# CMB-BNU/PloidyFrost

Hardware: AMD Instinct MI355X
Metric: unitigs/s through superbubble+SeqAlign (k=25, z=8) (higher is better)
Workload: dtype u64

## Files before the change

ploidyfrost_amd/csrc/pf_call.hip:

```cpp
#include "pf_call_kernels.hpp"
#include "pf_scan.hpp"

using namespace pf;

#define PF_HIP(call)                                                                         \
    do {                                                                                     \
        hipError_t e_ = (call);                                                              \
        if (e_ != hipSuccess) {                                                              \
            pf::CtxErr{ctx} = std::string(#call) + ": " + hipGetErrorString(e_);                   \
            return PF_ERR_HIP;                                                               \
        }                                                                                    \
    } while (0)

#define PF_TRY(call) do { const int s_ = (call); if (s_ != PF_OK) return s_; } while (0)

using namespace pf_call;

struct Need { DevBuf *buf; size_t bytes; };
static int need(pf_ctx *ctx, const char *who, std::initializer_list<Need> list) {
    for (const Need &n : list)
        if (!n.buf->ensure(n.bytes)) { pf::CtxErr{ctx} = std::string(who) + ": out of device memory"; return PF_ERR_HIP; }
    return PF_OK;
}

namespace pf {

void call_state_create(pf_ctx *ctx) { (void)state_of(ctx); }
void call_destroy(pf_ctx *ctx) {
    if (!ctx->call) return;
    ctx->call->release_all();
    delete ctx->call;
    ctx->call = nullptr;
}
void call_invalidate(pf_ctx *ctx) {
    if (!ctx->call) return;
    ctx->call->have_cov = false;
    ctx->call->have_state = false;
    ctx->call->n_sides = ctx->call->n_tasks = 0;
}

}

namespace pf {
int call_state_arrays(pf_ctx *ctx, uint8_t **flags, uint32_t **plus, uint32_t **minus) {
    if (!ctx->d_seq || !ctx->has_adj) { pf::CtxErr{ctx} = "T1 state: graph and adjacency first"; return PF_ERR_ARG; }
    CallState *S = state_of(ctx);
    const size_t N = ctx->N;
    if (!S->flags.ensure(N + 1) || !S->plus.ensure(N * 4) || !S->minus.ensure(N * 4)) { pf::CtxErr{ctx} = "T1 state: out of device memory"; return PF_ERR_HIP; }
    *flags = S->flags.as<uint8_t>();
    *plus = S->plus.as<uint32_t>();
    *minus = S->minus.as<uint32_t>();
    S->have_state = false;
    return PF_OK;
}
void call_state_resident(pf_ctx *ctx) {
    CallState *S = state_of(ctx);
    S->have_state = true;
    S->n_sides = S->n_tasks = 0;
}
}

extern "C" {

int pf_format_doubles(pf_ctx *ctx, const double *values, uint64_t n, char *text, uint8_t *len) {
    if (!ctx || (n && (!values || !text || !len))) return PF_ERR_ARG;
    if (n == 0) return PF_OK;
    PF_HIP(hipSetDevice(ctx->device));
    DevTmp<double> dx;
    DevTmp<char> dt;
    DevTmp<uint8_t> dl;
    PF_HIP(dx.alloc(n * 8));
    PF_HIP(dt.alloc(n * 32));
    PF_HIP(dl.alloc(n));
    PF_HIP(hipMemcpyAsync(dx.p, values, n * 8, hipMemcpyDefault, ctx->stream));
    k_format_doubles<<<(unsigned)((n + 255) / 256), 256, 0, ctx->stream>>>(dx.p, n, dt.p, dl.p);
    PF_HIP(hipGetLastError());
    PF_HIP(hipMemcpyAsync(text, dt.p, n * 32, hipMemcpyDefault, ctx->stream));
    PF_HIP(hipMemcpyAsync(len, dl.p, n, hipMemcpyDefault, ctx->stream));
    PF_HIP(hipStreamSynchronize(ctx->stream));
    return PF_OK;
}

int pf_call_set_state(pf_ctx *ctx, const uint8_t *flags, const uint32_t *plus, const uint32_t *minus) {
    if (!ctx || !flags || !plus || !minus) return PF_ERR_ARG;
    if (!ctx->d_seq || !ctx->has_adj) { pf::CtxErr{ctx} = "pf_call_set_state: graph and adjacency first"; return PF_ERR_ARG; }
    PF_HIP(hipSetDevice(ctx->device));
    CallState *S = state_of(ctx);
    const size_t N = ctx->N;
    if (!S->flags.ensure(N + 1) || !S->plus.ensure(N * 4) || !S->minus.ensure(N * 4)) { pf::CtxErr{ctx} = "pf_call_set_state: out of device memory"; return PF_ERR_HIP; }
    PF_HIP(hipMemcpyAsync(S->flags.p, flags, N, hipMemcpyDefault, ctx->stream));
    PF_HIP(hipMemcpyAsync(S->plus.p, plus, N * 4, hipMemcpyDefault, ctx->stream));
    PF_HIP(hipMemcpyAsync(S->minus.p, minus, N * 4, hipMemcpyDefault, ctx->stream));
    PF_HIP(hipStreamSynchronize(ctx->stream));
    S->have_state = true;
    S->n_sides = S->n_tasks = 0;
    return PF_OK;
}

int pf_call_get_state(pf_ctx *ctx, uint8_t *flags, uint32_t *plus, uint32_t *minus) {
    if (!ctx || !ctx->call) return PF_ERR_ARG;
    CallState *S = ctx->call;
    if (!S->have_state) { pf::CtxErr{ctx} = "pf_call_get_state: no T1 state on the device"; return PF_ERR_ARG; }
    PF_HIP(hipSetDevice(ctx->device));
    const size_t N = ctx->N;
    PF_HIP(hipStreamSynchronize(ctx->stream));
    if (flags) PF_HIP(hipMemcpy(flags, S->flags.p, N, hipMemcpyDeviceToHost));
    if (plus) PF_HIP(hipMemcpy(plus, S->plus.p, N * 4, hipMemcpyDeviceToHost));
    if (minus) PF_HIP(hipMemcpy(minus, S->minus.p, N * 4, hipMemcpyDeviceToHost));
    return PF_OK;
}

int pf_call_set_format(pf_ctx *ctx, int reference_mt) {
    if (!ctx) return PF_ERR_ARG;
    state_of(ctx)->mt_format = reference_mt != 0;
    return PF_OK;
}

int pf_superbubble_rows(pf_ctx *ctx, int colored_rule, uint64_t *n_rows, uint64_t *text_len) {
    if (!ctx || !n_rows || !text_len) return PF_ERR_ARG;
    CallState *S = ctx->call;
    if (!S || !S->have_state) { pf::CtxErr{ctx} = "pf_superbubble_rows: pf_call_set_state first"; return PF_ERR_ARG; }
    PF_HIP(hipSetDevice(ctx->device));
    hipStream_t st = ctx->stream;
    const uint32_t N = ctx->N;
    const size_t n1 = (size_t)N + 1;
    if (!S->sb_cnt.ensure(n1 * 4) || !S->sb_base.ensure(n1 * 4) || !S->sb_sizes.ensure(n1 * 4) || !S->sb_offs.ensure(n1 * 8)) {
        pf::CtxErr{ctx} = "pf_superbubble_rows: out of device memory";
        return PF_ERR_HIP;
    }
    SbArgs a;
    a.flags = S->flags.as<uint8_t>(); a.plus = S->plus.as<uint32_t>(); a.minus = S->minus.as<uint32_t>(); a.N = N; a.colored = colored_rule;
    a.first_id = S->mt_format ? 0u : 1u;
    a.row_base = S->sb_base.as<uint32_t>(); a.sizes = S->sb_sizes.as<uint32_t>(); a.offs = S->sb_offs.as<uint64_t>(); a.out = nullptr;
    const unsigned grid = (unsigned)((n1 + 255) / 256);
    k_sb_count<<<grid, 256, 0, st>>>(a, S->sb_cnt.as<uint32_t>());
    if (!S->scan_tmp.ensure(scan_scratch_bytes(n1))) { pf::CtxErr{ctx} = "pf_superbubble_rows: out of device memory"; return PF_ERR_HIP; }
    PF_HIP(scan_exclusive_u32(S->sb_cnt.as<uint32_t>(), S->sb_base.as<uint32_t>(), n1, S->scan_tmp.p, st));
    ctx_begin(ctx, PF_K_CALL_FORMAT);
    k_sb_format<false><<<grid, 256, 0, st>>>(a);
    ctx_end(ctx);
    PF_HIP(scan_exclusive_u32_u64(S->sb_sizes.as<uint32_t>(), S->sb_offs.as<uint64_t>(), n1, S->scan_tmp.p, st));
    uint32_t rows = 0;
    uint64_t len = 0;
    PF_HIP(hipMemcpyAsync(&rows, S->sb_base.as<uint32_t>() + N, 4, hipMemcpyDeviceToHost, st));
    PF_HIP(hipMemcpyAsync(&len, S->sb_offs.as<uint64_t>() + N, 8, hipMemcpyDeviceToHost, st));
    PF_HIP(hipStreamSynchronize(st));
    if (!S->sb_out.ensure(std::max<uint64_t>(len, 16))) { pf::CtxErr{ctx} = "pf_superbubble_rows: out of device memory"; return PF_ERR_HIP; }
    a.out = S->sb_out.as<char>();
    hipStream_t wst = S->copy_stream ? S->copy_stream : st;
    ctx_begin_on(ctx, PF_K_CALL_FORMAT, wst);
    k_sb_format<true><<<grid, 256, 0, wst>>>(a);
    ctx_end_on(ctx, wst);
    PF_HIP(hipGetLastError());
    if (wst == st) PF_HIP(hipStreamSynchronize(st));
    S->sb_len = len;
    *n_rows = rows;
    *text_len = len;
    return PF_OK;
}

int pf_superbubble_fetch(pf_ctx *ctx, char *dst, uint64_t len) {
    if (!ctx || !ctx->call || (len && !dst)) return PF_ERR_ARG;
    CallState *S = ctx->call;
    if (len > S->sb_len) return PF_ERR_ARG;
    if (len == 0) return PF_OK;
    if (hipSetDevice(ctx->device) != hipSuccess || !S->copy_stream) return PF_ERR_HIP;
    size_t tl_at = (size_t)-1;
    (void)ctx_begin_at(ctx, PF_K_COPY_TEXT, S->copy_stream, &tl_at);
    if (hipMemcpyAsync(dst, S->sb_out.p, (size_t)len, hipMemcpyDeviceToHost, S->copy_stream) != hipSuccess) return PF_ERR_HIP;
    ctx_end_at(ctx, tl_at, S->copy_stream);
    if (hipStreamSynchronize(S->copy_stream) != hipSuccess) return PF_ERR_HIP;
    return PF_OK;
}

int pf_call_set_colours(pf_ctx *ctx, uint32_t n_colors, const uint64_t *full_mask, const uint64_t *size_total, const uint32_t *part_first,
                        const uint32_t *part_colour, const uint64_t *part_word, const uint64_t *part_bits, uint64_t n_part, uint64_t n_words) {
    if (!ctx || !ctx->d_seq) { if (ctx) pf::CtxErr{ctx} = "pf_call_set_colours: graph first"; return PF_ERR_ARG; }
    PF_HIP(hipSetDevice(ctx->device));
    CallState *S = state_of(ctx);
    S->n_colors = 0;
    S->have_cov = false;
    if (!n_colors) return PF_OK;
    if (n_colors > PF_MAX_COLORS || n_colors != ctx->n_colors || !full_mask || !size_total || !part_first || (n_part && (!part_colour || !part_word)) ||
        (n_words && !part_bits)) {
        pf::CtxErr{ctx} = "pf_call_set_colours: the colour sets of every unitig, for the colours of the uploaded databases, are required";
        return PF_ERR_ARG;
    }
    const size_t N = ctx->N, CW = (n_colors + 63) / 64;
    if (!S->col_low.ensure((size_t)n_colors * 4) || !S->col_up.ensure((size_t)n_colors * 4) || !S->col_full.ensure(N * CW * 8) || !S->col_size.ensure(N * 8) ||
        !S->part_first.ensure((N + 1) * 4) || !S->part_colour.ensure((n_part + 1) * 4) || !S->part_word.ensure((n_part + 1) * 8) ||
        !S->part_bits.ensure((n_words + 1) * 8)) {
        pf::CtxErr{ctx} = "pf_call_set_colours: out of device memory";
        return PF_ERR_HIP;
    }
    hipStream_t st = ctx->stream;
    PF_HIP(hipMemsetAsync(S->col_low.p, 0, (size_t)n_colors * 4, st));
    PF_HIP(hipMemsetAsync(S->col_up.p, 0xFF, (size_t)n_colors * 4, st));
    PF_HIP(hipMemcpyAsync(S->col_full.p, full_mask, N * CW * 8, hipMemcpyDefault, st));
    PF_HIP(hipMemcpyAsync(S->col_size.p, size_total, N * 8, hipMemcpyDefault, st));
    PF_HIP(hipMemcpyAsync(S->part_first.p, part_first, (N + 1) * 4, hipMemcpyDefault, st));
    if (n_part) {
        PF_HIP(hipMemcpyAsync(S->part_colour.p, part_colour, n_part * 4, hipMemcpyDefault, st));
        PF_HIP(hipMemcpyAsync(S->part_word.p, part_word, n_part * 8, hipMemcpyDefault, st));
    }
    if (n_words) PF_HIP(hipMemcpyAsync(S->part_bits.p, part_bits, n_words * 8, hipMemcpyDefault, st));
    PF_HIP(hipStreamSynchronize(st));
    S->n_colors = n_colors;
    S->col_words = (uint32_t)CW;
    return PF_OK;
}

int pf_call_set_cutoffs(pf_ctx *ctx, uint32_t n_colors, const uint32_t *lower, const uint32_t *upper) {
    if (!ctx || !ctx->call || !ctx->call->n_colors || n_colors != ctx->call->n_colors || !lower || !upper) {
        if (ctx) pf::CtxErr{ctx} = "pf_call_set_cutoffs: pf_call_set_colours first; one (lower, upper) per colour";
        return PF_ERR_ARG;
    }
    PF_HIP(hipSetDevice(ctx->device));
    CallState *S = ctx->call;
    PF_HIP(hipMemcpyAsync(S->col_low.p, lower, (size_t)n_colors * 4, hipMemcpyDefault, ctx->stream));
    PF_HIP(hipMemcpyAsync(S->col_up.p, upper, (size_t)n_colors * 4, hipMemcpyDefault, ctx->stream));
    PF_HIP(hipStreamSynchronize(ctx->stream));
    return PF_OK;
}

int pf_call_coverage(pf_ctx *ctx) {
    if (ctx && ctx->call && ctx->call->n_colors) {
        if (!ctx->d_seq || !ctx->d_ctab) { pf::CtxErr{ctx} = "pf_call_coverage: graph and count tables first"; return PF_ERR_ARG; }
        PF_HIP(hipSetDevice(ctx->device));
        CallState *S = ctx->call;
        const size_t n = (size_t)ctx->N * S->n_colors;
        if (!S->ccov_sum.ensure(n * 8) || !S->ccov_min.ensure(n * 4) || !S->ccov_max.ensure(n * 4) || !S->ccov_miss.ensure(n)) {
            pf::CtxErr{ctx} = "pf_call_coverage: out of device memory";
            return PF_ERR_HIP;
        }
        const int st = pf_unitig_cov_colored(ctx, 0, ctx->N, S->ccov_sum.as<uint64_t>(), S->ccov_min.as<uint32_t>(), S->ccov_max.as<uint32_t>(), S->ccov_miss.as<uint8_t>());
        if (st != PF_OK) return st;
        S->per_strand = false;
        S->have_cov = true;
        return PF_OK;
    }
    if (!ctx || !ctx->d_seq || !ctx->d_tab) { if (ctx) pf::CtxErr{ctx} = "pf_call_coverage: graph and count table first"; return PF_ERR_ARG; }
    PF_HIP(hipSetDevice(ctx->device));
    CallState *S = state_of(ctx);
    const size_t N = ctx->N;
    const int slots = ctx->tab_exact ? 2 : 1;
    if (!S->cov_sum.ensure(N * slots * 8) || !S->cov_min.ensure(N * slots * 4) || !S->cov_miss.ensure(N * slots)) {
        pf::CtxErr{ctx} = "pf_call_coverage: out of device memory";
        return PF_ERR_HIP;
    }
    int st;
    if (!ctx->tab_exact) {
        st = pf_unitig_cov(ctx, 0, (uint32_t)N, S->cov_sum.as<uint64_t>(), S->cov_min.as<uint32_t>(), S->cov_miss.as<uint8_t>());
    } else {
        st = pf_unitig_cov_exact(ctx, 0, (uint32_t)N, 0, S->cov_sum.as<uint64_t>(), S->cov_min.as<uint32_t>(), S->cov_miss.as<uint8_t>());
        if (st == PF_OK || st == PF_ERR_MISSING_KMER)
            st = pf_unitig_cov_exact(ctx, 0, (uint32_t)N, 1, S->cov_sum.as<uint64_t>() + N, S->cov_min.as<uint32_t>() + N, S->cov_miss.as<uint8_t>() + N);
    }
    if (st != PF_OK && st != PF_ERR_MISSING_KMER) return st;
    S->per_strand = ctx->tab_exact;
    S->have_cov = true;
    return PF_OK;
}

int pf_call_scan(pf_ctx *ctx, uint32_t lower, uint32_t upper, uint64_t *n_sides) {
    if (!ctx || !n_sides) return PF_ERR_ARG;
    CallState *S = ctx->call;
    if (!S || !S->have_state || !S->have_cov) { pf::CtxErr{ctx} = "pf_call_scan: pf_call_set_state and pf_call_coverage first"; return PF_ERR_ARG; }
    PF_HIP(hipSetDevice(ctx->device));
    hipStream_t st = ctx->stream;
    const uint32_t N = ctx->N;
    if (!S->side_cnt.ensure(((size_t)N + 1) * 4) || !S->side_base.ensure(((size_t)N + 1) * 4)) { pf::CtxErr{ctx} = "pf_call_scan: out of device memory"; return PF_ERR_HIP; }
    k_call_count_sides<<<(N + 1 + 255) / 256, 256, 0, st>>>(S->flags.as<uint8_t>(), N, S->side_cnt.as<uint32_t>());
    if (!S->scan_tmp.ensure(scan_scratch_bytes((uint64_t)N + 1))) { pf::CtxErr{ctx} = "pf_call_scan: out of device memory"; return PF_ERR_HIP; }
    PF_HIP(scan_exclusive_u32(S->side_cnt.as<uint32_t>(), S->side_base.as<uint32_t>(), (uint64_t)N + 1, S->scan_tmp.p, st));
    uint32_t total = 0;
    PF_HIP(hipMemcpyAsync(&total, S->side_base.as<uint32_t>() + N, 4, hipMemcpyDeviceToHost, st));
    PF_HIP(hipStreamSynchronize(st));
    S->n_sides = total;
    S->n_tasks = 0;
    S->low = lower;
    S->up = upper;
    *n_sides = total;
    if (total == 0) return PF_OK;
    if (!S->sides.ensure((size_t)total * sizeof(pf_call_side)) || !S->ctask.ensure((size_t)total * sizeof(CallTask)) ||
        !S->target.ensure((size_t)total * 4)) {
        pf::CtxErr{ctx} = "pf_call_scan: out of device memory";
        return PF_ERR_HIP;
    }
    ScanArgs a;
    a.flags = S->flags.as<uint8_t>(); a.plus = S->plus.as<uint32_t>(); a.minus = S->minus.as<uint32_t>();
    a.succ = ctx->d_succ; a.pred = ctx->d_pred; a.seq = ctx->d_seq; a.off = ctx->d_off; a.len = ctx->d_len; a.N = N; a.k = ctx->k;
    a.cov_sum = S->cov_sum.as<uint64_t>(); a.cov_min = S->cov_min.as<uint32_t>(); a.cov_miss = S->cov_miss.as<uint8_t>();
    a.per_strand = S->per_strand; a.low = lower; a.up = upper;
    a.side_base = S->side_base.as<uint32_t>(); a.sides = S->sides.as<pf_call_side>(); a.tasks = S->ctask.as<CallTask>();
    a.target = S->target.as<uint32_t>();
    a.n_colors = S->n_colors;
    a.ccov_sum = S->ccov_sum.as<uint64_t>(); a.ccov_min = S->ccov_min.as<uint32_t>(); a.ccov_max = S->ccov_max.as<uint32_t>(); a.ccov_miss = S->ccov_miss.as<uint8_t>();
    a.clow = S->col_low.as<uint32_t>(); a.cup = S->col_up.as<uint32_t>(); a.full = S->col_full.as<uint64_t>(); a.cwords = S->col_words; a.size_total = S->col_size.as<uint64_t>();
    ctx_begin(ctx, PF_K_CALL_SCAN);
    if (S->n_colors) k_call_sides<true><<<(N + 255) / 256, 256, 0, st>>>(a);
    else k_call_sides<false><<<(N + 255) / 256, 256, 0, st>>>(a);
    ctx_end(ctx);
    ctx_units(ctx, PF_K_CALL_SCAN, N);
    PF_HIP(hipGetLastError());
    return PF_OK;
}

int pf_call_resolve(pf_ctx *ctx, uint64_t *n_bubbles, uint32_t *err, uint32_t *err_unitig) {
    if (!ctx || !ctx->call || !n_bubbles || !err || !err_unitig) return PF_ERR_ARG;
    CallState *S = ctx->call;
    *n_bubbles = 0;
    *err = 0;
    *err_unitig = 0;
    S->n_tasks = 0;
    const uint64_t n = S->n_sides;
    if (n == 0) return PF_OK;
    PF_HIP(hipSetDevice(ctx->device));
    hipStream_t st = ctx->stream;
    if (!S->pending.ensure(n * 4) || !S->killed.ensure(n) || !S->rstate.ensure(n) || !S->rflag.ensure(n * 4) || !S->rsmall.ensure(64) ||
        !S->kept.ensure(n * 4)) {
        pf::CtxErr{ctx} = "pf_call_resolve: out of device memory";
        return PF_ERR_HIP;
    }
    PF_HIP(hipMemsetAsync(S->pending.p, 0, n * 4, st));
    PF_HIP(hipMemsetAsync(S->killed.p, 0, n, st));
    PF_HIP(hipMemsetAsync(S->rstate.p, 0, n, st));
    unsigned int *small = S->rsmall.as<unsigned int>();
    ResolveArgs a;
    a.sides = S->sides.as<pf_call_side>(); a.target = S->target.as<uint32_t>(); a.n = (uint32_t)n; a.pending = S->pending.as<int>();
    a.killed = S->killed.as<uint8_t>(); a.state = S->rstate.as<uint8_t>(); a.flag = S->rflag.as<uint32_t>();
    a.undecided = small; a.first_err = small + 1;
    const unsigned int init[3] = {0, 0xFFFFFFFFu, 0};
    PF_HIP(hipMemcpyAsync(small, init, 12, hipMemcpyHostToDevice, st));
    const unsigned grid = (unsigned)((n + 255) / 256);
    k_call_pending<<<grid, 256, 0, st>>>(a);
    for (uint64_t round = 0;; ++round) {
        if (round > n + 2) { pf::CtxErr{ctx} = "pf_call_resolve: the driver pass does not settle"; return PF_ERR_ARG; }
        k_call_resolve<<<grid, 256, 0, st>>>(a);
        PF_HIP(hipMemsetAsync(small, 0, 4, st));
        k_call_resolve<<<grid, 256, 0, st>>>(a);
        unsigned int h[2];
        PF_HIP(hipMemcpyAsync(h, small, 8, hipMemcpyDeviceToHost, st));
        PF_HIP(hipStreamSynchronize(st));
        if (h[1] != 0xFFFFFFFFu && h[0] == 0) {
            pf_call_side bad;
            PF_HIP(hipMemcpy(&bad, S->sides.as<pf_call_side>() + h[1], sizeof(bad), hipMemcpyDeviceToHost));
            *err = bad.err;
            *err_unitig = bad.err_unitig;
            return PF_OK;
        }
        if (h[0] == 0) break;
    }
    if (!S->scan_tmp.ensure(scan_scratch_bytes(n))) { pf::CtxErr{ctx} = "pf_call_resolve: out of device memory"; return PF_ERR_HIP; }
    PF_HIP(select_flagged_u32(S->rflag.as<uint32_t>(), S->kept.as<uint32_t>(), small + 2, nullptr, n, S->scan_tmp.p, st));
    unsigned int sel = 0;
    PF_HIP(hipMemcpyAsync(&sel, small + 2, 4, hipMemcpyDeviceToHost, st));
    PF_HIP(hipStreamSynchronize(st));
    S->n_tasks = sel;
    *n_bubbles = sel;
    return PF_OK;
}

int pf_call_sides(pf_ctx *ctx, pf_call_side *out, uint64_t cap) {
    if (!ctx || !ctx->call) return PF_ERR_ARG;
    CallState *S = ctx->call;
    if (cap < S->n_sides || (S->n_sides && !out)) return PF_ERR_OVERFLOW;
    if (S->n_sides == 0) return PF_OK;
    PF_HIP(hipSetDevice(ctx->device));
    PF_HIP(hipMemcpyAsync(out, S->sides.p, (size_t)S->n_sides * sizeof(pf_call_side), hipMemcpyDefault, ctx->stream));
    PF_HIP(hipStreamSynchronize(ctx->stream));
    return PF_OK;
}

int pf_call_select(pf_ctx *ctx, const uint32_t *side_index, uint64_t n_tasks) {
    if (!ctx || !ctx->call || (n_tasks && !side_index)) return PF_ERR_ARG;
    CallState *S = ctx->call;
    if (n_tasks > S->n_sides) { pf::CtxErr{ctx} = "pf_call_select: more bubbles than open sides"; return PF_ERR_ARG; }
    PF_HIP(hipSetDevice(ctx->device));
    if (!S->kept.ensure(std::max<size_t>(n_tasks, 1) * 4)) { pf::CtxErr{ctx} = "pf_call_select: out of device memory"; return PF_ERR_HIP; }
    if (n_tasks) PF_HIP(hipMemcpyAsync(S->kept.p, side_index, (size_t)n_tasks * 4, hipMemcpyDefault, ctx->stream));
    PF_HIP(hipStreamSynchronize(ctx->stream));
    S->n_tasks = n_tasks;
    return PF_OK;
}

}

namespace {

int ensure_batch_buffers(pf_ctx *ctx, const char *who, CallState::AlignWork &W, CallState::AlignOut &O, uint32_t nb) {
    const size_t list = (size_t)nb * 4;
    return need(ctx, who, {{&W.counters, sizeof(CallCounters)}, {&W.btask, (size_t)nb * sizeof(pf_bubble_task)}, {&W.queues, (size_t)NQ * list},
                           {&W.blist, list}, {&W.slist, list}, {&W.plist, list}, {&W.plist2, list}, {&W.klist, list}, {&W.klist_b, list}, {&W.has, list},
                           {&O.res, (size_t)nb * sizeof(pf_bubble_result)}, {&O.sv_off, (size_t)nb * 8}, {&O.vc, list}});
}

int ensure_wave_scratch(pf_ctx *ctx, const char *who, CallState::AlignWork &W, const CallGrids &g, uint32_t depth, bool stack_tier, bool pair_tier) {
    PF_TRY(need(ctx, who, {{&W.paths_scr, paths_per_wave(depth) * g.paths}}));
    if (stack_tier) PF_TRY(need(ctx, who, {{&W.stack_scr, stack_scratch_bytes() * g.stack}}));
    if (pair_tier) PF_TRY(need(ctx, who, {{&W.pair_scr, PairGeom<PAIR_MAX>::scratch_bytes * g.pair}}));
    return PF_OK;
}

int ensure_pools(pf_ctx *ctx, const char *who, CallState::AlignWork &W, CallState::AlignOut &O, uint32_t nb, const BatchPools &p) {
    PF_TRY(need(ctx, who, {{&W.bpath, p.path_entries(nb) * sizeof(pf_bubble_path)}, {&W.ptext, p.path_text}, {&O.otext, p.row_text},
                           {&O.osites, p.sites * sizeof(pf_bubble_site)}, {&O.ogroups, p.groups}, {&O.oilen, p.ilen * 4}}));
    if (p.walk) PF_TRY(need(ctx, who, {{&W.walk_pool, p.walk * 4}, {&W.walk_off, (size_t)nb * 8}}));
    return PF_OK;
}

int ensure_lane_streams(pf_ctx *ctx, CallState::AlignWork &W, int lane) {
    if (lane != 0 && !W.stream) { PF_HIP(lane_stream_create(&W.stream, lane)); W.own_stream = true; }
    if (!W.side_stream) {
        PF_HIP(lane_stream_create(&W.side_stream, lane));
        PF_HIP(hipEventCreateWithFlags(&W.ev_prep, hipEventDisableTiming));
        PF_HIP(hipEventCreateWithFlags(&W.ev_paths, hipEventDisableTiming));
    }
    return PF_OK;
}

int stats_begin(pf_ctx *ctx, DevTmp<unsigned long long> &prof, size_t words, hipStream_t st, unsigned long long **arg) {
    PF_HIP(prof.alloc(words * 8));
    PF_HIP(hipMemsetAsync(prof.p, 0, words * 8, st));
    *arg = prof.p;
    return PF_OK;
}
int print_pair_stats(pf_ctx *ctx, const DevTmp<unsigned long long> &prof) {
    unsigned long long h[8];
    PF_HIP(hipMemcpy(h, prof.p, 64, hipMemcpyDeviceToHost));
    fprintf(stderr, "[k_call_pair] %llu wavefront rounds; lane-0 ticks (10 ns): decode %llu fill %llu traceback %llu classify %llu publish %llu\n", h[5],
            h[0], h[1], h[2], h[3], h[4]);
    return PF_OK;
}
int print_sites_stats(pf_ctx *ctx, const DevTmp<unsigned long long> &prof, int grid, hipStream_t st) {
    PF_HIP(hipStreamSynchronize(st));
    std::vector<unsigned long long> h((size_t)grid * 6);
    PF_HIP(hipMemcpy(h.data(), prof.p, h.size() * 8, hipMemcpyDeviceToHost));
    unsigned long long sum[6] = {0, 0, 0, 0, 0, 0}, mx = 0;
    for (int w = 0; w < grid; ++w) {
        for (int x = 0; x < 6; ++x) sum[x] += h[(size_t)w * 6 + x];
        mx = std::max(mx, h[(size_t)w * 6]);
    }
    fprintf(stderr, "[k_call_sites] %d wavefronts, %llu bubbles; ticks (10 ns) per wavefront: total %.0f (max %llu) = pop + load %.0f, strings %.0f, ranks + probes %.0f, groups %.0f\n",
            grid, sum[5], (double)sum[0] / grid, mx, (double)sum[1] / grid, (double)sum[2] / grid, (double)sum[3] / grid, (double)sum[4] / grid);
    return PF_OK;
}

int env_int(const char *name, int otherwise) { const char *e = getenv(name); return e ? atoi(e) : otherwise; }

struct AlignTrace {
    const bool on = getenv("PF_TRACE_ALIGN") != nullptr;
    const std::chrono::steady_clock::time_point t_enter = std::chrono::steady_clock::now();
    void stage(const char *what) const {
        if (on) fprintf(stderr, "[pf_call_align]   %-34s %.2f ms\n", what, std::chrono::duration<double>(std::chrono::steady_clock::now() - t_enter).count() * 1e3);
    }
};

struct AlignCall {
    static constexpr const char *who = "pf_call_run";
    pf_ctx *const ctx; CallState *const S;
    CallState::AlignWork &W; CallState::AlignOut &O;
    const int lane; const uint64_t t0; const uint32_t nb;
    const double match, mismatch, gap;
    const AlignTrace trace;
    const bool snp_ok = snp_shortcut_scores(match, mismatch, gap);
    const bool pair_tier = std::fabs(match) < 1e5 && std::fabs(mismatch) < 1e5 && std::fabs(gap) < 1e5;
    const bool pair_integral = match == std::floor(match) && mismatch == std::floor(mismatch) && gap == std::floor(gap);
    const bool stack_tier = stack_scores(match, mismatch, gap);
    const int stack_ok = stack_tier ? std::max(1, std::min(3, env_int("PF_STACK_LEVEL", 1))) : 0;
    const int paths_force_scratch = env_int("PF_PATHS_SCRATCH", 0) ? 1 : 0;
    const CallGrids grids = call_grids(ctx->n_cu);
    const uint32_t depth;
    hipStream_t st = nullptr;
    CallCounters *d_cnt = nullptr;
    BatchRef batch = {};
    GraphSeq graph = {};
    CallLists lists = {};
    RowPools pools;
    BatchPools cap = {};
    PathArgs ph = {};
    PairArgs pr = {};
    int attempt = 0;
    CallCounters hc = {};
    unsigned long long heads[4] = {0, 0, 0, 0};
    uint64_t n_jobs = 0;
    uint32_t n_called = 0;
    size_t tl_at = (size_t)-1;

    AlignCall(pf_ctx *c, int lane_, uint64_t t0_, uint32_t nb_, uint32_t complex_size, double m, double d, double g)
        : ctx(c), S(c->call), W(c->call->work[lane_]), O(c->call->lane[lane_]), lane(lane_), t0(t0_), nb(nb_), match(m), mismatch(d), gap(g), depth(depth_cap(complex_size)) {}

    void tbegin(int kernel, hipStream_t s) { (void)ctx_begin_at(ctx, kernel, s, &tl_at); }
    void tend(hipStream_t s) { ctx_end_at(ctx, tl_at, s); }

    int prepare() {
        PF_TRY(ensure_lane_streams(ctx, W, lane));
        st = lane == 0 ? ctx->stream : W.stream;
        for (hipEvent_t e : O.read_ev) if (e) PF_HIP(hipStreamWaitEvent(st, e, 0));
        PF_TRY(ensure_batch_buffers(ctx, who, W, O, nb));
        PF_TRY(ensure_wave_scratch(ctx, who, W, grids, depth, stack_tier, pair_tier));
        if (W.mlist_cap < MANY_LIST_MIN) W.mlist_cap = MANY_LIST_MIN;
        PF_TRY(need(ctx, who, {{&W.mlist, (size_t)W.mlist_cap * 4}}));
        d_cnt = W.counters.as<CallCounters>();
        batch = BatchRef{S->ctask.as<CallTask>(), S->kept.as<uint32_t>(), t0, nb};
        graph = GraphSeq{ctx->d_seq, ctx->d_off, ctx->d_len};
        lists = CallLists{W.queues.as<uint32_t>(), W.blist.as<uint32_t>(), W.slist.as<uint32_t>(), W.plist.as<uint32_t>(), W.plist2.as<uint32_t>(), W.klist.as<uint32_t>(), W.klist_b.as<uint32_t>(), nb};
        trace.stage("lists and scratch");
        return PF_OK;
    }

    int size_pools() {
        LearntPools l;
        l.path_pool = S->path_pool; l.path_text = S->text_pool; l.row_text = S->otext_cap; l.sites = S->osites_cap; l.groups = S->ogroups_cap; l.ilen = S->oilen_cap;
        l.walk = W.walk_cap;
        cap = batch_pools(nb, grids, l, S->n_colors != 0);
        PF_TRY(ensure_pools(ctx, who, W, O, nb, cap));
        unsigned long long *d_heads = bubble_pool_heads(ctx, lane);
        if (!d_heads) return PF_ERR_HIP;
        pools = RowPools{O.res.as<pf_bubble_result>(), O.otext.as<char>(), cap.row_text, O.osites.as<pf_bubble_site>(), cap.sites, O.ogroups.as<uint8_t>(), cap.groups,
                         O.oilen.as<uint32_t>(), cap.ilen, d_heads};
        PF_HIP(hipMemsetAsync(d_cnt, 0, sizeof(CallCounters), st));
        PF_HIP(hipMemsetAsync(d_heads, 0, 32, st));
        return PF_OK;
    }

    int launch_tiers() {
        PrepArgs pa;
        pa.batch = batch; pa.len = graph.len; pa.btask = W.btask.as<pf_bubble_task>(); pa.bpath = W.bpath.as<pf_bubble_path>(); pa.res = pools.res;
        pa.lists = lists; pa.snp_ok = snp_ok ? 1 : 0; pa.pair_ok = pair_tier ? 1 : 0; pa.stack_ok = stack_ok; pa.cnt = d_cnt;
        tbegin(PF_K_CALL_PREP, st);
        k_call_prep<<<(nb + 255) / 256, 256, 0, st>>>(pa);
        tend(st);
        hipStream_t pst = W.side_stream;
        PF_HIP(hipEventRecord(W.ev_prep, st));
        PF_HIP(hipStreamWaitEvent(pst, W.ev_prep, 0));
        ph = PathArgs{};
        ph.batch = batch; ph.blist = lists.blist; ph.succ = ctx->d_succ; ph.graph = graph; ph.k = ctx->k; ph.depth_cap = depth;
        ph.scratch = W.paths_scr.as<uint8_t>(); ph.scratch_per_wave = paths_per_wave(depth); ph.force_scratch = paths_force_scratch;
        ph.max_paths = MAX_PATHS; ph.n_list = &d_cnt->n_branching; ph.mlist = W.mlist.as<uint32_t>(); ph.mlist_cap = W.mlist_cap;
        ph.walk_pool = S->n_colors ? W.walk_pool.as<uint32_t>() : nullptr; ph.walk_off = W.walk_off.as<uint64_t>(); ph.walk_cap = cap.walk;
        ph.btask = pa.btask; ph.bpath = pa.bpath; ph.path_cap = cap.path_pool; ph.text = W.ptext.as<char>(); ph.text_cap = cap.path_text;
        ph.queues = lists.queues; ph.klist = lists.klist_b; ph.stack_ok = stack_ok; ph.cnt = d_cnt;
        tbegin(PF_K_CALL_PATHS, pst);
        k_call_paths<false><<<grids.paths, 64, 0, pst>>>(ph);
        tend(pst);
        PF_HIP(hipEventRecord(W.ev_paths, pst));
        if (snp_ok) {
            SnpArgs sn;
            sn.batch = batch; sn.slist = lists.slist; sn.graph = graph; sn.out = pools; sn.lists = lists; sn.pair_ok = pa.pair_ok; sn.stack_ok = stack_ok; sn.cnt = d_cnt;
            tbegin(PF_K_CALL_SNP, st);
            k_call_snp<<<(nb + 255) / 256, 256, 0, st>>>(sn);
            tend(st);
        }
        StackArgs sk;
        if (stack_tier) {
            sk.list = lists.klist; sk.n_list = &d_cnt->n_stack; sk.scratch = W.stack_scr.as<uint8_t>(); sk.pair_ok = pa.pair_ok;
            sk.btask = pa.btask; sk.bpath = pa.bpath; sk.ptext = W.ptext.as<char>(); sk.graph = graph;
            sk.M = (int)match; sk.D = (int)mismatch; sk.G = (int)gap;
            sk.out = pools; sk.lists = lists; sk.cnt = d_cnt;
            tbegin(PF_K_CALL_STACK, st);
            k_call_stack<<<grids.stack, 64, 0, st>>>(sk);
            tend(st);
        }
        if (pair_tier) {
            pr = PairArgs{};
            pr.batch = batch; pr.graph = graph; pr.M = match; pr.D = mismatch; pr.G = gap; pr.Mi = (int)match; pr.Di = (int)mismatch; pr.Gi = (int)gap;
            pr.list = lists.plist; pr.n_list = &d_cnt->n_pair; pr.n_done = &d_cnt->n_pair_done;
            pr.scratch = W.pair_scr.as<uint8_t>(); pr.out = pools; pr.lists = lists; pr.cnt = d_cnt;
            static const bool pair_stats = getenv("PF_PAIR_STATS") != nullptr;
            DevTmp<unsigned long long> prof;
            if (pair_stats) PF_TRY(stats_begin(ctx, prof, 8, st, &pr.prof));
            tbegin(PF_K_CALL_PAIR, st);
            if (pair_integral) k_call_pair<PAIR_MAX, true><<<grids.pair, 64, 0, st>>>(pr);
            else k_call_pair<PAIR_MAX, false><<<grids.pair, 64, 0, st>>>(pr);
            tend(st);
            if (pair_stats) PF_TRY(print_pair_stats(ctx, prof));
            pr.prof = nullptr;
        }
        PF_HIP(hipStreamWaitEvent(st, W.ev_paths, 0));
        if (stack_tier) {
            sk.list = lists.klist_b; sk.n_list = &d_cnt->n_stack_b; sk.pair_ok = 0;
            tbegin(PF_K_CALL_STACK, st);
            k_call_stack<<<grids.stack, 64, 0, st>>>(sk);
            tend(st);
        }
        return PF_OK;
    }

    int read_counters() {
        PF_HIP(hipGetLastError());
        PF_HIP(hipMemcpyAsync(&hc, d_cnt, sizeof(hc), hipMemcpyDeviceToHost, st));
        PF_HIP(hipStreamSynchronize(st));
        return PF_OK;
    }

    int launch_pair_tier2() {
        if (!pair_tier || !hc.n_pair2) return PF_OK;
        PairArgs p2 = pr;
        p2.list = lists.plist2; p2.n_list = &d_cnt->n_pair2; p2.n_done = &d_cnt->n_pair2_done;
        const uint32_t tier2_min = (uint32_t)env_int("PF_PAIR2_MIN", 0);
        if (hc.n_pair2 < (tier2_min ? tier2_min : pair2_min(ctx->n_cu))) {
            k_call_pair2_reroute<<<(hc.n_pair2 + 255) / 256, 256, 0, st>>>(p2);
        } else {
            const int g2 = call_pair2_grid(hc.n_pair2, grids);
            PF_TRY(need(ctx, who, {{&W.pair_scr2, PairGeom<PAIR_MAX2>::scratch_bytes * g2}}));
            p2.scratch = W.pair_scr2.as<uint8_t>();
            tbegin(PF_K_CALL_PAIR, st);
            if (pair_integral) k_call_pair<PAIR_MAX2, true><<<g2, 64, 0, st>>>(p2);
            else k_call_pair<PAIR_MAX2, false><<<g2, 64, 0, st>>>(p2);
            tend(st);
        }
        return read_counters();
    }

    void note_units() const {
        ctx_units(ctx, PF_K_CALL_PREP, nb);
        if (snp_ok) ctx_units(ctx, PF_K_CALL_SNP, hc.n_snp);
        if (pair_tier) ctx_units(ctx, PF_K_CALL_PAIR, hc.n_pair + hc.n_pair2);
        if (stack_tier) ctx_units(ctx, PF_K_CALL_STACK, hc.n_stack + hc.n_stack_b);
        ctx_units(ctx, PF_K_CALL_PATHS, hc.n_branching);
        if (trace.on) fprintf(stderr, "[pf_call_align] bubbles of more than 255 walks: %u, err %u\n", hc.n_many, hc.err);
    }

    int launch_paths_big(bool *retry) {
        if (!hc.n_many || (hc.err & ERR_WALK)) return PF_OK;
        if (hc.n_many > W.mlist_cap) {
            W.mlist_cap = grown_many(hc.n_many);
            *retry = true;
            return need(ctx, who, {{&W.mlist, (size_t)W.mlist_cap * 4}});
        }
        const int big_grid = paths_big_grid(hc.n_many);
        const uint64_t big_per_wave = paths_big_per_wave(depth, PATHS_BIG);
        PF_TRY(need(ctx, who, {{&W.paths_big_scr, big_per_wave * big_grid}}));
        PathArgs pb = ph;
        pb.blist = W.mlist.as<uint32_t>(); pb.n_list = &d_cnt->n_many; pb.max_paths = PATHS_BIG; pb.mlist = nullptr; pb.mlist_cap = 0;
        pb.scratch = W.paths_big_scr.as<uint8_t>(); pb.scratch_per_wave = big_per_wave;
        tbegin(PF_K_CALL_PATHS, st);
        k_call_paths<true><<<big_grid, 64, 0, st>>>(pb);
        tend(st);
        return read_counters();
    }

    int accept_walks(bool *retry) {
        if (hc.err & ERR_WALK) {
            char where[96];
            snprintf(where, sizeof where, " (superbubble from unitig %u%c to unitig %u%c)", (hc.err_entrance >> 1) + 1, (hc.err_entrance & 1) ? '-' : '+',
                     (hc.err_exit >> 1) + 1, (hc.err_exit & 1) ? '-' : '+');
            pf::CtxErr{ctx} = std::string(hc.err & ERR_MANY_PATHS ? "pf_call_run: a bubble has more than 65535 paths" : "pf_call_run: a bubble is deeper than the complex size allows") + where;
            return PF_ERR_ARG;
        }
        amax(S->otext_cap, cap.row_text); amax(S->osites_cap, cap.sites);
        amax(S->ogroups_cap, cap.groups); amax(S->oilen_cap, cap.ilen);
        amax(S->path_pool, cap.path_pool);
        amax(S->text_pool, cap.path_text);
        const uint64_t rows_need = row_text_need(hc.text_head, hc.n_branching, nb);
        if (trace.on)
            fprintf(stderr, "[pf_call_align] attempt %d: %u bubbles, path pool %llu of %llu, path text %llu of %llu, rows text cap %llu (needs %llu)\n", attempt, nb,
                    (unsigned long long)hc.path_head, (unsigned long long)cap.path_pool, (unsigned long long)hc.text_head, (unsigned long long)cap.path_text,
                    (unsigned long long)cap.row_text, (unsigned long long)rows_need);
        if (hc.path_head > cap.path_pool || hc.text_head > cap.path_text || hc.walk_head > cap.walk) {
            amax(S->path_pool, grown(hc.path_head, 1024));
            amax(S->text_pool, grown(hc.text_head, 4096));
            if (S->n_colors) W.walk_cap = std::max<uint64_t>(W.walk_cap, grown(hc.walk_head, 1024));
            *retry = true;
            return PF_OK;
        }
        if (S->n_colors) W.walk_cap = std::max(W.walk_cap, cap.walk);
        if (cap.row_text < rows_need) {
            amax(S->otext_cap, rows_need + rows_need / 16 + 4096);
            *retry = true;
        }
        return PF_OK;
    }

    int run_bubble(bool *retry) {
        n_jobs = 0;
        for (int x = 0; x < NQ; ++x) n_jobs += hc.q_n[x];
        PF_TRY(need(ctx, who, {{&W.scan_tmp2, std::max<size_t>((size_t)n_jobs, 1) * 4}}));
        uint32_t *d_idx = W.scan_tmp2.as<uint32_t>();
        size_t at = 0;
        for (int x = 0; x < NQ; ++x) {
            if (!hc.q_n[x]) continue;
            PF_HIP(hipMemcpyAsync(d_idx + at, W.queues.as<uint32_t>() + (size_t)x * nb, (size_t)hc.q_n[x] * 4, hipMemcpyDeviceToDevice, st));
            at += hc.q_n[x];
        }
        BubbleLaunch BL;
        BL.text = W.ptext.as<char>(); BL.paths = W.bpath.as<pf_bubble_path>(); BL.tasks = W.btask.as<pf_bubble_task>();
        BL.n_tasks = nb; BL.idx = d_idx;
        for (int c = 0; c <= kBubLdsClasses; ++c) BL.n_cls[c] = hc.q_n[2 * c] + hc.q_n[2 * c + 1];
        BL.max_need = hc.max_need; BL.retry_need = hc.retry_need;
        BL.match = match; BL.mismatch = mismatch; BL.gap = gap;
        BL.out = pools;
        BL.keep_heads = true;
        BL.lane = lane; BL.stream = st;
        trace.stage("K-BUBBLE launching");
        const int bst = bubble_launch(ctx, BL, heads);
        trace.stage("K-BUBBLE done");
        if (trace.on)
            fprintf(stderr, "[pf_call_align] attempt %d: K-BUBBLE status %d, pools text %llu of %llu, sites %llu of %llu, groups %llu of %llu, indel lengths %llu of %llu\n", attempt, bst,
                    heads[0], (unsigned long long)cap.row_text, heads[1], (unsigned long long)cap.sites, heads[2], (unsigned long long)cap.groups, heads[3], (unsigned long long)cap.ilen);
        if (bst == PF_ERR_OVERFLOW && (heads[0] > cap.row_text || heads[1] > cap.sites || heads[2] > cap.groups || heads[3] > cap.ilen)) {
            amax(S->otext_cap, heads[0] + heads[0] / 8);
            amax(S->osites_cap, heads[1] + heads[1] / 8);
            amax(S->ogroups_cap, heads[2] + heads[2] / 8);
            amax(S->oilen_cap, heads[3] + heads[3] / 8);
            *retry = true;
            return PF_OK;
        }
        return bst;
    }

    int number_called() {
        k_call_has<<<(nb + 255) / 256, 256, 0, st>>>(O.res.as<pf_bubble_result>(), nb, W.has.as<uint32_t>());
        PF_TRY(need(ctx, who, {{&W.scan_tmp, scan_scratch_bytes(nb)}}));
        PF_HIP(scan_inclusive_u32(W.has.as<uint32_t>(), O.vc.as<uint32_t>(), nb, W.scan_tmp.p, st));
        PF_HIP(hipMemcpyAsync(&n_called, O.vc.as<uint32_t>() + (nb - 1), 4, hipMemcpyDeviceToHost, st));
        return PF_OK;
    }

    SiteArgs site_args(uint32_t ks, uint64_t rows_cap, uint64_t per_wave, uint64_t sv_cap) const {
        SiteArgs sa;
        sa.batch = batch; sa.blist = lists.blist; sa.res = pools.res; sa.otext = pools.otext; sa.osites = pools.osites; sa.ogroups = pools.ogroups;
        sa.k = ctx->k; sa.tab = ctx->d_tab; sa.mask = ctx->tab_cap - 1; sa.one_strand = ctx->tab_one_strand; sa.tab_exact = ctx->tab_exact;
        sa.low = S->low; sa.up = S->up; sa.ks = ks; sa.rows_cap = (uint32_t)rows_cap;
        sa.scratch = W.sites_scr.as<uint8_t>(); sa.scratch_per_wave = per_wave; sa.sv_off = O.sv_off.as<uint64_t>();
        sa.sv = O.sv.as<double>(); sa.sv_cap = sv_cap; sa.cnt = d_cnt; sa.prof = nullptr;
        sa.n_colors = S->n_colors;
        sa.ctab = CTab{ctx->d_ctab, ctx->ctab_cap - 1, ctx->ctab_line_bytes}; sa.c_one_strand = ctx->ctab_one_strand; sa.unread = ctx->d_unread;
        sa.clow = S->col_low.as<uint32_t>(); sa.cup = S->col_up.as<uint32_t>(); sa.full = S->col_full.as<uint64_t>(); sa.cwords = S->col_words;
        sa.part_first = S->part_first.as<uint32_t>(); sa.part_colour = S->part_colour.as<uint32_t>(); sa.part_word = S->part_word.as<uint64_t>();
        sa.part_bits = S->part_bits.as<uint64_t>(); sa.walk_pool = W.walk_pool.as<uint32_t>(); sa.walk_off = W.walk_off.as<uint64_t>();
        sa.graph = graph;
        return sa;
    }

    int launch_sites(SiteArgs &sa, int grid) {
        static const bool sites_stats = getenv("PF_SITES_STATS") != nullptr;
        DevTmp<unsigned long long> prof;
        if (sites_stats) PF_TRY(stats_begin(ctx, prof, (size_t)grid * 6, st, &sa.prof));
        PF_HIP(hipMemsetAsync(&d_cnt->sites_next, 0, 4, st));
        PF_HIP(hipMemsetAsync(&d_cnt->sv_head, 0, 8, st));
        PF_HIP(hipMemsetAsync(&d_cnt->site_strings, 0, 8, st));
        tbegin(PF_K_CALL_SITES, st);
        if (sa.n_colors) k_call_sites<true><<<grid, 64, 0, st>>>(sa);
        else k_call_sites<false><<<grid, 64, 0, st>>>(sa);
        tend(st);
        ctx_units(ctx, PF_K_CALL_SITES, hc.n_branching);
        if (sites_stats) { PF_HIP(hipGetLastError()); PF_TRY(print_sites_stats(ctx, prof, grid, st)); }
        return read_counters();
    }

    int run_sites() {
        uint32_t KS = std::max<uint32_t>(first_site_string(ctx->k), S->sites_ks.load());
        const uint32_t C = S->n_colors;
        const uint64_t rows_cap = sites_rows_cap(hc.max_rows);
        for (int sv_attempt = 0, ks_attempt = 0;;) {
            const uint64_t per_wave = sites_per_wave(rows_cap, KS, C, S->col_words);
            const int grid = call_sites_grid(hc.n_branching, grids, per_wave);
            const uint64_t sv_cap = site_values_cap(C, hc.n_branching, grid, S->sv_pool);
            PF_TRY(need(ctx, who, {{&W.sites_scr, per_wave * grid}, {&O.sv, sv_cap * 8}}));
            SiteArgs sa = site_args(KS, rows_cap, per_wave, sv_cap);
            PF_TRY(launch_sites(sa, grid));
            if (hc.err & ERR_SITE_LONG) {
                if (++ks_attempt > 3 || hc.ks_need <= KS) { pf::CtxErr{ctx} = "pf_call_run: the room for a site string does not converge"; return PF_ERR_OVERFLOW; }
                KS = grown_site_string(hc.ks_need);
                amax(S->sites_ks, KS);
                hc.err = 0; hc.ks_need = 0;
                PF_HIP(hipMemsetAsync(&d_cnt->err, 0, 4, st));
                PF_HIP(hipMemsetAsync(&d_cnt->ks_need, 0, 4, st));
                continue;
            }
            if (hc.err & ERR_MISSING_KMER) { pf::CtxErr{ctx} = "CDBG::readCov(): a kmer of a site string can not found ."; return PF_ERR_MISSING_KMER; }
            if (hc.err & ERR_SITE_ROW) { pf::CtxErr{ctx} = "CDBG::PloidyEstimation(): a site string runs past the end of an aligned row (the reference terminates here: std::out_of_range from substr, src/CDBG.cpp:1478-1590)"; return PF_ERR_ARG; }
            if (hc.err & ERR_SITE_UNITIG) { pf::CtxErr{ctx} = "CCDBG::PloidyEstimation(): a site string does not start on a unitig of its bubble"; return PF_ERR_ARG; }
            if (hc.sv_head > sv_cap) {
                if (sv_attempt++ >= 2) { pf::CtxErr{ctx} = "pf_call_run: site value pool does not converge"; return PF_ERR_OVERFLOW; }
                amax(S->sv_pool, grown(hc.sv_head, 1024));
                continue;
            }
            amax(S->sv_pool, sv_cap);
            return PF_OK;
        }
    }
};

}

extern "C" {

int pf_call_align_lane(pf_ctx *ctx, int lane, uint64_t t0, uint64_t t1, uint32_t complex_size, double match, double mismatch, double gap,
                       pf_call_result *out) {
    if (!ctx || !out || lane < 0 || lane >= PF_CALL_LANES) return PF_ERR_ARG;
    CallState *S = ctx->call;
    if (!S || t0 > t1 || t1 > S->n_tasks) { pf::CtxErr{ctx} = "pf_call_align: range outside the selection"; return PF_ERR_ARG; }
    memset(out, 0, sizeof(*out));
    CallState::AlignOut &O = S->lane[lane];
    O.nb = 0;
    O.t0 = t0;
    O.cur = pf_call_result{};
    if (t1 == t0) return PF_OK;
    if (t1 - t0 > (1u << 24)) { pf::CtxErr{ctx} = "pf_call_align: at most 2^24 bubbles per batch"; return PF_ERR_ARG; }
    PF_HIP(hipSetDevice(ctx->device));
    AlignCall A(ctx, lane, t0, (uint32_t)(t1 - t0), complex_size, match, mismatch, gap);
    PF_TRY(A.prepare());
    for (A.attempt = 0;; ++A.attempt) {
        if (A.attempt > 5) { pf::CtxErr{ctx} = "pf_call_align: pools do not converge"; return PF_ERR_OVERFLOW; }
        bool retry = false;
        PF_TRY(A.size_pools());
        PF_TRY(A.launch_tiers());
        PF_TRY(A.read_counters());
        A.trace.stage("K-PREP .. K-STACK done");
        PF_TRY(A.launch_pair_tier2());
        A.note_units();
        PF_TRY(A.launch_paths_big(&retry));
        if (!retry) PF_TRY(A.accept_walks(&retry));
        if (!retry) PF_TRY(A.run_bubble(&retry));
        if (!retry) break;
    }
    const CallCounters &hc = A.hc;
    out->n_branching = hc.n_branching;
    out->align_jobs = A.n_jobs + hc.n_snp_done + hc.n_pair_done + hc.n_pair2_done + hc.n_stack_done;
    out->snp_jobs = hc.n_snp_done; out->pair_jobs = hc.n_pair_done + hc.n_pair2_done; out->wave_jobs = A.n_jobs; out->stack_jobs = hc.n_stack_done;
    PF_TRY(A.number_called());
    if (hc.n_branching) {
        PF_TRY(A.run_sites());
    } else {
        PF_TRY(need(ctx, A.who, {{&O.sv, 16}}));
        PF_HIP(hipStreamSynchronize(A.st));
    }
    out->site_strings = hc.site_strings;
    A.trace.stage("K-SITES done");
    out->n_called = A.n_called;
    O.nb = A.nb;
    O.cur = *out;
    for (int x = 0; x < 4; ++x) O.used[x] = A.heads[x];
    O.used[4] = hc.n_branching ? hc.sv_head : 0;
    return PF_OK;
}

int pf_call_peek(pf_ctx *ctx, int lane, pf_call_bubble *bubbles, pf_bubble_result *results, uint64_t *sv_off, uint64_t bubble_cap, char *text,
                 pf_bubble_site *sites, uint8_t *groups, uint32_t *ilen, double *sv, const uint64_t cap[5], uint64_t used[6]) {
    if (!ctx || lane < 0 || lane >= PF_CALL_LANES || !used) return PF_ERR_ARG;
    CallState *S = ctx->call;
    if (!S) { pf::CtxErr{ctx} = "pf_call_peek: pf_call_align first"; return PF_ERR_ARG; }
    if (S->n_colors) { pf::CtxErr{ctx} = "pf_call_peek: the single-sample path's view (a colored site holds one value per colour and group)"; return PF_ERR_ARG; }
    const CallState::AlignOut &O = S->lane[lane];
    used[0] = O.nb;
    for (int x = 0; x < 5; ++x) used[x + 1] = O.used[x];
    if (!O.nb) return PF_OK;
    if (!bubbles && !results && !text && !sites && !groups && !ilen && !sv && !sv_off) return PF_OK;
    if (bubble_cap < O.nb || !cap) return PF_ERR_ARG;
    for (int x = 0; x < 5; ++x)
        if (cap[x] < O.used[x]) return PF_ERR_ARG;
    PF_HIP(hipSetDevice(ctx->device));
    if (bubbles) {
        std::vector<uint32_t> kept(O.nb);
        PF_HIP(hipMemcpy(kept.data(), S->kept.as<uint32_t>() + O.t0, (size_t)O.nb * 4, hipMemcpyDeviceToHost));
        std::vector<CallTask> ct(S->n_sides);
        if (S->n_sides) PF_HIP(hipMemcpy(ct.data(), S->ctask.p, (size_t)S->n_sides * sizeof(CallTask), hipMemcpyDeviceToHost));
        for (uint32_t j = 0; j < O.nb; ++j) {
            const CallTask &t = ct[kept[j]];
            pf_call_bubble &b = bubbles[j];
            b.entrance_ov = t.entrance_ov; b.exit_ov = t.exit_ov; b.strict = t.strict; b.n_inner = t.n_inner;
            for (int x = 0; x < 4; ++x) { b.inner[x] = t.inner[x]; b.cov[x] = t.cov[x]; }
            b.core_mean = t.core_mean; b.cov_sum = t.cov_sum;
        }
    }
    if (results) PF_HIP(hipMemcpy(results, O.res.p, (size_t)O.nb * sizeof(pf_bubble_result), hipMemcpyDeviceToHost));
    if (sv_off) PF_HIP(hipMemcpy(sv_off, O.sv_off.p, (size_t)O.nb * 8, hipMemcpyDeviceToHost));
    if (text && O.used[0]) PF_HIP(hipMemcpy(text, O.otext.p, O.used[0], hipMemcpyDeviceToHost));
    if (sites && O.used[1]) PF_HIP(hipMemcpy(sites, O.osites.p, O.used[1] * sizeof(pf_bubble_site), hipMemcpyDeviceToHost));
    if (groups && O.used[2]) PF_HIP(hipMemcpy(groups, O.ogroups.p, O.used[2], hipMemcpyDeviceToHost));
    if (ilen && O.used[3]) PF_HIP(hipMemcpy(ilen, O.oilen.p, O.used[3] * 4, hipMemcpyDeviceToHost));
    if (sv && O.used[4]) PF_HIP(hipMemcpy(sv, O.sv.p, O.used[4] * 8, hipMemcpyDeviceToHost));
    return PF_OK;
}

int pf_call_reserve_lanes(pf_ctx *ctx, uint64_t nb64, uint32_t complex_size, int n_lanes) {
    if (!ctx || nb64 == 0 || n_lanes < 1 || n_lanes > PF_CALL_LANES) return PF_ERR_ARG;
    CallState *S = state_of(ctx);
    PF_HIP(hipSetDevice(ctx->device));
    const uint32_t nb = (uint32_t)std::min<uint64_t>(nb64, 1u << 24);
    const char *who = "pf_call_reserve";
    const CallGrids grids = call_grids(ctx->n_cu);
    DevLoadTrace trace;
    for (int lane = 0; lane < n_lanes; ++lane) {
        CallState::AlignWork &W = S->work[lane];
        CallState::AlignOut &O = S->lane[lane];
        PF_TRY(ensure_batch_buffers(ctx, who, W, O, nb));
        PF_TRY(ensure_wave_scratch(ctx, who, W, grids, depth_cap(complex_size), true, true));
        PF_TRY(ensure_pools(ctx, who, W, O, nb, batch_pools(nb, grids, LearntPools{}, false)));
        PF_TRY(need(ctx, who, {{&W.scan_tmp2, reserve_job_index_bytes(nb)}, {&W.sites_scr, sites_per_wave(256, first_site_string(31), 0, 1) * grids.sites},
                               {&O.sv, reserve_site_values(nb, grids) * 8}}));
        trace.mark("reserve: a lane's buffers");
        PF_TRY(ensure_lane_streams(ctx, W, lane));
        trace.mark("reserve: a lane's streams and events");
        PF_TRY(bubble_reserve(ctx, nb, lane));
        trace.mark("reserve: K-BUBBLE's workspaces and first launches");
    }
    return PF_OK;
}

int pf_call_reserve(pf_ctx *ctx, uint64_t nb64, uint32_t complex_size) { return pf_call_reserve_lanes(ctx, nb64, complex_size, 2); }

int pf_call_align(pf_ctx *ctx, uint64_t t0, uint64_t t1, uint32_t complex_size, double match, double mismatch, double gap,
                  pf_call_result *out) {
    return pf_call_align_lane(ctx, 0, t0, t1, complex_size, match, mismatch, gap, out);
}

static int text_work_of(pf_ctx *ctx, pf::CallState *S, int which, uint32_t nb) {
    pf::CallState::TextWork &T = S->text[which];
    if (!T.stream) {
        int least = 0, greatest = 0;
        PF_HIP(hipDeviceGetStreamPriorityRange(&least, &greatest));
        PF_HIP(hipStreamCreateWithPriority(&T.stream, hipStreamNonBlocking, greatest));
    }
    return need(ctx, "pf_call_text", {{&T.sizes, (size_t)N_INT * (nb + 1) * 4}, {&T.offs, ((size_t)N_INT * (nb + 1) + 1) * 8}, {&T.totals, 16 * 8},
                                      {&T.tcounters, sizeof(CallCounters)}, {&T.tscan, scan_scratch_bytes((uint64_t)N_INT * (nb + 1))}});
}

int pf_call_reserve_text(pf_ctx *ctx, uint64_t piece_bubbles) {
    if (!ctx || piece_bubbles == 0) return PF_ERR_ARG;
    pf::CallState *S = state_of(ctx);
    PF_HIP(hipSetDevice(ctx->device));
    const uint32_t nb = (uint32_t)std::min<uint64_t>(piece_bubbles, 1u << 24);
    for (int which = 0; which < 2; ++which) { const int ts = text_work_of(ctx, S, which, nb); if (ts != PF_OK) return ts; }
    for (int slab = 0; slab < PF_CALL_SLABS; ++slab) PF_TRY(need(ctx, "pf_call_text", {{&S->out[slab], (11ull * 31 + 40) * nb}}));
    for (int which = 0; which < 2; ++which) {
        pf::CallState::TextWork &T = S->text[which];
        FmtArgs fa;
        memset(&fa, 0, sizeof(fa));
        fa.sizes = T.sizes.as<uint32_t>(); fa.offs = T.offs.as<uint64_t>(); fa.cnt = T.tcounters.as<CallCounters>();
        if (S->n_colors) { k_call_format<false, true><<<1, FMT_BLOCK, 0, T.stream>>>(fa); k_call_format<true, true><<<1, FMT_BLOCK, 0, T.stream>>>(fa); }
        else { k_call_format<false, false><<<1, FMT_BLOCK, 0, T.stream>>>(fa); k_call_format<true, false><<<1, FMT_BLOCK, 0, T.stream>>>(fa); }
        PF_HIP(hipGetLastError());
        PF_HIP(hipStreamSynchronize(T.stream));
    }
    return PF_OK;
}

static int call_text_impl(pf_ctx *ctx, int lane, int slab, uint64_t first, uint64_t count, uint64_t var_count_base, pf_call_result *out, bool sizes_only) {
    if (!ctx || !out || slab < 0 || slab >= PF_CALL_SLABS || lane < 0 || lane >= PF_CALL_LANES) return PF_ERR_ARG;
    CallState *S = ctx->call;
    if (!S) return PF_ERR_ARG;
    CallState::AlignOut &O = S->lane[lane];
    if (first + count > O.nb) { pf::CtxErr{ctx} = "pf_call_text_range: range outside the aligned batch"; return PF_ERR_ARG; }
    if (S->n_colors && S->mt_format) { pf::CtxErr{ctx} = "pf_call_text_range: the -t > 1 format is the single-sample path's"; return PF_ERR_ARG; }
    if (!sizes_only)
        for (int s = 0; s < N_STREAMS; ++s) S->out_len[slab][s] = 0;
    *out = O.cur;
    out->n_called = 0;
    if (count == 0) return PF_OK;
    PF_HIP(hipSetDevice(ctx->device));
    const bool trace_stages = getenv("PF_TRACE_ALIGN") != nullptr;
    const auto t_enter = std::chrono::steady_clock::now();
    auto ta = [&](const char *what) {
        if (trace_stages) fprintf(stderr, "[pf_call_text]    %-34s %.2f ms\n", what, std::chrono::duration<double>(std::chrono::steady_clock::now() - t_enter).count() * 1e3);
    };
    const uint32_t nb = (uint32_t)count;
    const int which = sizes_only ? 0 : (slab & 1);
    { const int ts = text_work_of(ctx, S, which, nb); if (ts != PF_OK) return ts; }
    CallState::TextWork &T = S->text[which];
    hipStream_t st = T.stream;
    const uint64_t t0 = O.t0;
    uint32_t vc_edge[2] = {0, 0};
    PF_HIP(hipMemcpyAsync(&vc_edge[1], O.vc.as<uint32_t>() + (first + count - 1), 4, hipMemcpyDeviceToHost, st));
    if (first) PF_HIP(hipMemcpyAsync(&vc_edge[0], O.vc.as<uint32_t>() + (first - 1), 4, hipMemcpyDeviceToHost, st));
    CallCounters *d_cnt = T.tcounters.as<CallCounters>();
    CallCounters hc;
    const size_t n_sizes = (size_t)N_INT * (nb + 1);
    ta("stream and size tables");
    PF_HIP(hipMemsetAsync(&d_cnt->allele[0], 0, 6 * 8, st));
    FmtArgs fa;
    fa.ct = S->ctask.as<CallTask>(); fa.kept = S->kept.as<uint32_t>(); fa.t0 = t0; fa.j0 = (uint32_t)first; fa.nb = nb;
    fa.res = O.res.as<pf_bubble_result>();
    fa.otext = O.otext.as<char>(); fa.osites = O.osites.as<pf_bubble_site>(); fa.ogroups = O.ogroups.as<uint8_t>();
    fa.oilen = O.oilen.as<uint32_t>(); fa.sv_off = O.sv_off.as<uint64_t>(); fa.sv = O.sv.as<double>(); fa.vc = O.vc.as<uint32_t>();
    fa.vc_base = var_count_base; fa.mt = S->mt_format ? 1 : 0; fa.len = ctx->d_len; fa.sizes = T.sizes.as<uint32_t>(); fa.offs = T.offs.as<uint64_t>(); fa.cnt = d_cnt;
    for (int s = 0; s < N_INT; ++s) fa.out[s] = nullptr;
    fa.packed = S->pack_alignseq ? 1 : 0;
    size_t at = 0;
    ctx_begin_at(ctx, PF_K_CALL_FORMAT, st, &at);
    fa.n_colors = S->n_colors; fa.N = ctx->N; fa.k = ctx->k; fa.full = S->col_full.as<uint64_t>(); fa.cwords = S->col_words; fa.ccov_sum = S->ccov_sum.as<uint64_t>();
    if (S->n_colors) k_call_format<false, true><<<(nb + 1 + FMT_BLOCK - 1) / FMT_BLOCK, FMT_BLOCK, 0, st>>>(fa);
    else k_call_format<false, false><<<(nb + 1 + FMT_BLOCK - 1) / FMT_BLOCK, FMT_BLOCK, 0, st>>>(fa);
    ctx_end_at(ctx, at, st);
    PF_HIP(scan_exclusive_u32_u64(T.sizes.as<uint32_t>(), T.offs.as<uint64_t>(), n_sizes, T.tscan.p, st));
    k_call_totals<<<1, 64, 0, st>>>(T.offs.as<uint64_t>(), T.sizes.as<uint32_t>(), nb, T.totals.as<uint64_t>());
    uint64_t totals[N_INT + 1] = {};
    PF_HIP(hipMemcpyAsync(totals, T.totals.p, N_INT * 8, hipMemcpyDeviceToHost, st));
    PF_HIP(hipMemcpyAsync(&hc, d_cnt, sizeof(hc), hipMemcpyDeviceToHost, st));
    PF_HIP(hipStreamSynchronize(st));
    out->n_called = vc_edge[1] - vc_edge[0];
    const uint64_t packed_len = (fa.packed && totals[PF_OUT_ALIGNSEQ]) ? alnpack_index_bytes(nb) + totals[S_PACK] : 0;
    auto slab_len = [&](int s) { return (s == PF_OUT_ALIGNSEQ && fa.packed) ? packed_len : totals[s]; };
    out->alignseq_packed_len = packed_len;
    uint64_t all = 0;
    for (int s = 0; s < N_STREAMS; ++s) all += slab_len(s);
    if (sizes_only) {
        for (int s = 0; s < N_STREAMS; ++s) out->text_len[s] = totals[s];
        for (int x = 0; x < 4; ++x) out->allele[x] = hc.allele[x];
        out->core_cov = hc.core_cov;
        out->core_num = hc.core_num;
        return PF_OK;
    }
    ta("sizes counted");
    PF_TRY(need(ctx, "pf_call_text", {{&S->out[slab], std::max<uint64_t>(all, 16)}}));
    ta("slab taken");
    all = 0;
    for (int s = 0; s < N_STREAMS; ++s) {
        fa.out[s] = S->out[slab].as<char>() + all;
        S->out_off[slab][s] = all;
        S->out_len[slab][s] = slab_len(s);
        out->text_len[s] = totals[s];
        all += slab_len(s);
    }
    if (fa.packed) { fa.out[S_PACK] = fa.out[PF_OUT_ALIGNSEQ]; fa.out[PF_OUT_ALIGNSEQ] = nullptr; }
    if (S->model.read_ev[slab]) PF_HIP(hipStreamWaitEvent(st, S->model.read_ev[slab], 0));
    ctx_begin_at(ctx, PF_K_CALL_FORMAT, st, &at);
    if (S->n_colors) k_call_format<true, true><<<(nb + FMT_BLOCK - 1) / FMT_BLOCK, FMT_BLOCK, 0, st>>>(fa);
    else k_call_format<true, false><<<(nb + FMT_BLOCK - 1) / FMT_BLOCK, FMT_BLOCK, 0, st>>>(fa);
    ctx_end_at(ctx, at, st);
    ctx_units(ctx, PF_K_CALL_FORMAT, nb);
    PF_HIP(hipGetLastError());
    S->fetch_base[slab] = S->out[slab].as<char>();
    S->nib[slab] = false;
    out->numeric_packed = 0;
    for (int s = 0; s < N_STREAMS; ++s) { S->txt_off[slab][s] = S->out_off[slab][s]; S->txt_len[slab][s] = S->out_len[slab][s]; }
    if (S->pack_numeric) {
        uint64_t foff[N_STREAMS], flen[N_STREAMS], fall = 0;
        for (int s = 0; s < N_STREAMS; ++s) {
            flen[s] = s == PF_OUT_ALIGNSEQ ? ((slab_len(s) + 15) & ~15ull) : PF_NUMERIC_PACKED_LEN(totals[s]);
            foff[s] = fall;
            fall += flen[s];
        }
        PF_TRY(need(ctx, "pf_call_text", {{&S->outp[slab], fall + 16}}));
        char *pb = S->outp[slab].as<char>();
        PF_HIP(hipMemsetAsync(pb + fall, 0, 16, st));
        if (slab_len(PF_OUT_ALIGNSEQ))
            PF_HIP(hipMemcpyAsync(pb + foff[PF_OUT_ALIGNSEQ], S->out[slab].as<char>() + S->txt_off[slab][PF_OUT_ALIGNSEQ], (size_t)slab_len(PF_OUT_ALIGNSEQ), hipMemcpyDeviceToDevice, st));
        NibArgs na;
        int x = 0;
        uint64_t units = 0;
        for (int s = 0; s < N_STREAMS; ++s) {
            if (s == PF_OUT_ALIGNSEQ) continue;
            na.src[x] = S->out[slab].as<char>() + S->txt_off[slab][s];
            na.dst[x] = reinterpret_cast<uint8_t *>(pb + foff[s]);
            na.len[x] = totals[s];
            na.unit0[x] = units;
            na.stream[x] = (uint32_t)s;
            units += (totals[s] + 15) / 16;
            ++x;
        }
        na.unit0[NIB_STREAMS] = units;
        na.flag = reinterpret_cast<uint32_t *>(pb + fall);
        if (units) k_text_nibbles<<<(unsigned)((units + 255) / 256), 256, 0, st>>>(na);
        PF_HIP(hipGetLastError());
        for (int s = 0; s < N_STREAMS; ++s) { S->out_off[slab][s] = foff[s]; S->out_len[slab][s] = flen[s]; }
        S->fetch_base[slab] = pb;
        S->nib[slab] = true;
        out->numeric_packed = 1;
    }
    if (!S->text_ev[slab]) PF_HIP(hipEventCreateWithFlags(&S->text_ev[slab], hipEventDisableTiming));
    PF_HIP(hipEventRecord(S->text_ev[slab], st));
    if (!O.read_ev[which]) PF_HIP(hipEventCreateWithFlags(&O.read_ev[which], hipEventDisableTiming));
    PF_HIP(hipEventRecord(O.read_ev[which], st));
    for (int x = 0; x < 4; ++x) out->allele[x] = hc.allele[x];
    out->core_cov = hc.core_cov;
    out->core_num = hc.core_num;
    return PF_OK;
}

int pf_call_set_numeric_packed(pf_ctx *ctx, int on) {
    if (!ctx) return PF_ERR_ARG;
    CallState *S = state_of(ctx);
    if (!S) return PF_ERR_HIP;
    S->pack_numeric = on != 0;
    return PF_OK;
}

int pf_call_fetch_text(pf_ctx *ctx, int slab, int stream, char *dst, uint64_t len) {
    if (!ctx || !ctx->call || slab < 0 || slab >= PF_CALL_SLABS || stream < 0 || stream >= N_STREAMS) return PF_ERR_ARG;
    CallState *S = ctx->call;
    if (len > S->txt_len[slab][stream] || (len && !dst)) return PF_ERR_ARG;
    if (len == 0) return PF_OK;
    if (hipSetDevice(ctx->device) != hipSuccess || !S->copy_stream) return PF_ERR_HIP;
    if (S->text_ev[slab] && hipStreamWaitEvent(S->copy_stream, S->text_ev[slab], 0) != hipSuccess) return PF_ERR_HIP;
    if (hipMemcpyAsync(dst, S->out[slab].as<char>() + S->txt_off[slab][stream], (size_t)len, hipMemcpyDeviceToHost, S->copy_stream) != hipSuccess) return PF_ERR_HIP;
    if (hipStreamSynchronize(S->copy_stream) != hipSuccess) return PF_ERR_HIP;
    S->fetched_bytes.fetch_add(len, std::memory_order_relaxed);
    return PF_OK;
}

int pf_call_set_alignseq_packed(pf_ctx *ctx, int on) {
    if (!ctx) return PF_ERR_ARG;
    CallState *S = state_of(ctx);
    if (!S) return PF_ERR_HIP;
    S->pack_alignseq = on != 0;
    return PF_OK;
}

int pf_call_text_range_lane(pf_ctx *ctx, int lane, int slab, uint64_t first, uint64_t count, uint64_t var_count_base, pf_call_result *out) {
    return call_text_impl(ctx, lane, slab, first, count, var_count_base, out, false);
}

int pf_call_text_sizes(pf_ctx *ctx, int lane, uint64_t first, uint64_t count, uint64_t var_count_base, pf_call_result *out) {
    return call_text_impl(ctx, lane, 0, first, count, var_count_base, out, true);
}

int pf_call_text_range(pf_ctx *ctx, int slab, uint64_t first, uint64_t count, uint64_t var_count_base, pf_call_result *out) {
    return pf_call_text_range_lane(ctx, 0, slab, first, count, var_count_base, out);
}

int pf_call_text(pf_ctx *ctx, int slab, uint64_t var_count_base, pf_call_result *out) {
    if (!ctx || !ctx->call) return PF_ERR_ARG;
    const int st = pf_call_text_range(ctx, slab, 0, ctx->call->lane[0].nb, var_count_base, out);
    if (st == PF_OK) out->n_called = ctx->call->lane[0].cur.n_called;
    return st;
}

int pf_call_run(pf_ctx *ctx, int slab, uint64_t t0, uint64_t t1, uint64_t var_count_base, uint32_t complex_size, double match,
                double mismatch, double gap, pf_call_result *out) {
    const int st = pf_call_align(ctx, t0, t1, complex_size, match, mismatch, gap, out);
    if (st != PF_OK) return st;
    return pf_call_text(ctx, slab, var_count_base, out);
}

int pf_call_fetch(pf_ctx *ctx, int slab, int stream, char *dst, uint64_t len) {
    if (!ctx || !ctx->call || slab < 0 || slab >= PF_CALL_SLABS || stream < 0 || stream >= N_STREAMS) return PF_ERR_ARG;
    CallState *S = ctx->call;
    if (len > S->out_len[slab][stream] || (len && !dst)) return PF_ERR_ARG;
    if (len == 0) return PF_OK;
    if (hipSetDevice(ctx->device) != hipSuccess) return PF_ERR_HIP;
    if (!S->copy_stream) return PF_ERR_HIP;
    if (S->text_ev[slab] && hipStreamWaitEvent(S->copy_stream, S->text_ev[slab], 0) != hipSuccess) return PF_ERR_HIP;
    if (hipMemcpyAsync(dst, S->fetch_base[slab] + S->out_off[slab][stream], (size_t)len, hipMemcpyDeviceToHost, S->copy_stream) != hipSuccess) return PF_ERR_HIP;
    if (hipStreamSynchronize(S->copy_stream) != hipSuccess) return PF_ERR_HIP;
    S->fetched_bytes.fetch_add(len, std::memory_order_relaxed);
    return PF_OK;
}

int pf_call_fetch_slab(pf_ctx *ctx, int slab, char *dst, const uint64_t *len) {
    if (!ctx || !ctx->call || slab < 0 || slab >= PF_CALL_SLABS || !len) return PF_ERR_ARG;
    CallState *S = ctx->call;
    if (hipSetDevice(ctx->device) != hipSuccess) return PF_ERR_HIP;
    if (!S->copy_stream) return PF_ERR_HIP;
    if (S->text_ev[slab] && hipStreamWaitEvent(S->copy_stream, S->text_ev[slab], 0) != hipSuccess) return PF_ERR_HIP;
    uint64_t at = 0;
    bool whole = true;
    for (int s = 0; s < N_STREAMS; ++s) {
        if (len[s] > S->out_len[slab][s] || (len[s] && !dst)) return PF_ERR_ARG;
        whole = whole && len[s] == S->out_len[slab][s];
        at += len[s];
    }
    size_t tl_at = (size_t)-1;
    (void)ctx_begin_at(ctx, PF_K_COPY_TEXT, S->copy_stream, &tl_at);
    if (whole) {
        const uint64_t tail = S->nib[slab] ? 16 : 0;
        if (at + tail && hipMemcpyAsync(dst, S->fetch_base[slab], (size_t)(at + tail), hipMemcpyDeviceToHost, S->copy_stream) != hipSuccess) return PF_ERR_HIP;
    } else {
        at = 0;
        for (int s = 0; s < N_STREAMS; ++s) {
            if (len[s] && hipMemcpyAsync(dst + at, S->fetch_base[slab] + S->out_off[slab][s], (size_t)len[s], hipMemcpyDeviceToHost, S->copy_stream) != hipSuccess)
                return PF_ERR_HIP;
            at += len[s];
        }
    }
    ctx_end_at(ctx, tl_at, S->copy_stream);
    if (hipStreamSynchronize(S->copy_stream) != hipSuccess) return PF_ERR_HIP;
    S->fetched_bytes.fetch_add(at, std::memory_order_relaxed);
    return PF_OK;
}

int pf_call_fetch_range(pf_ctx *ctx, int slab, uint64_t first_byte, char *dst, uint64_t len, int slot) {
    if (!ctx || !ctx->call || slab < 0 || slab >= PF_CALL_SLABS || slot < 0 || slot > 1 || (len && !dst)) return PF_ERR_ARG;
    CallState *S = ctx->call;
    uint64_t all = 0;
    for (int s = 0; s < N_STREAMS; ++s) all += S->out_len[slab][s];
    if (first_byte + len > all) return PF_ERR_ARG;
    if (hipSetDevice(ctx->device) != hipSuccess || !S->copy_stream) return PF_ERR_HIP;
    if (!S->fetch_ev[slot] && hipEventCreateWithFlags(&S->fetch_ev[slot], hipEventDisableTiming) != hipSuccess) return PF_ERR_HIP;
    if (S->text_ev[slab] && hipStreamWaitEvent(S->copy_stream, S->text_ev[slab], 0) != hipSuccess) return PF_ERR_HIP;
    size_t tl_at = (size_t)-1;
    (void)ctx_begin_at(ctx, PF_K_COPY_TEXT, S->copy_stream, &tl_at);
    if (len && hipMemcpyAsync(dst, S->fetch_base[slab] + first_byte, (size_t)len, hipMemcpyDeviceToHost, S->copy_stream) != hipSuccess) return PF_ERR_HIP;
    ctx_end_at(ctx, tl_at, S->copy_stream);
    if (hipEventRecord(S->fetch_ev[slot], S->copy_stream) != hipSuccess) return PF_ERR_HIP;
    S->fetched_bytes.fetch_add(len, std::memory_order_relaxed);
    return PF_OK;
}

int pf_call_fetch_wait(pf_ctx *ctx, int slot) {
    if (!ctx || !ctx->call || slot < 0 || slot > 1 || !ctx->call->fetch_ev[slot]) return PF_ERR_ARG;
    if (hipSetDevice(ctx->device) != hipSuccess) return PF_ERR_HIP;
    return hipEventSynchronize(ctx->call->fetch_ev[slot]) == hipSuccess ? PF_OK : PF_ERR_HIP;
}

}
```

ploidyfrost_amd/csrc/pf_call_plan.hpp:

```cpp
#pragma once

#include <algorithm>
#include <cstdint>

namespace pf_call {

constexpr uint32_t FIRST_ROW_TEXT = 384, FIRST_SITES = 4, FIRST_GROUPS = 12, FIRST_ILEN = 2, FIRST_PATH_TEXT = 64;

constexpr int paths_per_cu = 16, sites_per_cu = 16, pair_per_cu = 12, pair2_per_cu = 4, stack_per_cu = 8;

struct CallGrids {
    int paths, sites, pair, pair2, stack;
};
inline CallGrids call_grids(int n_cu) { return {n_cu * paths_per_cu, n_cu * sites_per_cu, n_cu * pair_per_cu, n_cu * pair2_per_cu, n_cu * stack_per_cu}; }

inline uint64_t round_up(uint64_t x, uint64_t to) { return (x + to - 1) & ~(to - 1); }
inline uint64_t grown(uint64_t need, uint64_t slack) { return need + need / 8 + slack; }

inline uint32_t depth_cap(uint32_t complex_size) { return std::max<uint32_t>(complex_size + 4, 16); }
inline uint64_t paths_stack_bytes(uint32_t depth) { return (10ull * depth + 4) * 4; }
inline uint64_t paths_per_wave(uint32_t depth) { return round_up(256 * 8 + 256 * 4 + paths_stack_bytes(depth), 256); }
inline uint64_t paths_big_per_wave(uint32_t depth, uint32_t max_paths) { return round_up(round_up(paths_stack_bytes(depth), 8) + ((uint64_t)max_paths + 1) * 12, 256); }
inline int paths_big_grid(uint32_t n_many) { return (int)std::min<uint32_t>(n_many, 32); }
constexpr uint32_t MANY_LIST_MIN = 4096;
inline uint32_t grown_many(uint32_t n_many) { return n_many + n_many / 8 + 64; }

inline int call_pair2_grid(uint32_t n_pair2, const CallGrids &g) { return (int)std::min<uint32_t>((n_pair2 + 63) / 64, (uint32_t)g.pair2); }
inline uint32_t pair2_min(int n_cu) { return (uint32_t)n_cu * 32u; }

inline uint32_t first_site_string(int k) { return (uint32_t)(2 * k + 64); }
inline uint32_t grown_site_string(uint32_t ks_need) { return (ks_need + 63u) & ~63u; }
inline uint64_t sites_rows_cap(uint32_t max_rows) { return std::max<uint64_t>(256, round_up(max_rows, 64)); }
inline uint64_t sites_per_wave(uint64_t rows_cap, uint64_t ks, uint32_t n_colors, uint32_t col_words) {
    return round_up(2 * rows_cap * ks + rows_cap * (4 + 4 + 4 + 1 + 1 + 8) + (n_colors ? rows_cap * (16ull * col_words + 8ull * n_colors + 1) : 0), 256);
}
inline int call_sites_grid(uint32_t n_branching, const CallGrids &g, uint64_t per_wave) {
    return (int)std::max<uint64_t>(1, std::min<uint64_t>(std::min<uint32_t>(n_branching, (uint32_t)g.sites), (2ull << 30) / per_wave));
}
inline uint64_t site_values_cap(uint32_t n_colors, uint32_t n_branching, int sites_grid, uint64_t learnt) {
    return std::max<uint64_t>(learnt, 8ull * std::max<uint32_t>(n_colors, 1) * n_branching + 1024ull * sites_grid + 1024);
}

struct LearntPools {
    uint64_t path_pool = 0, path_text = 0, row_text = 0, sites = 0, groups = 0, ilen = 0, walk = 0;
};
struct BatchPools {
    uint64_t path_pool;
    uint64_t path_text;
    uint64_t row_text, sites, groups, ilen;
    uint64_t walk;
    uint64_t path_entries(uint32_t nb) const { return 4ull * nb + path_pool; }
};
inline BatchPools batch_pools(uint32_t nb, const CallGrids &g, const LearntPools &l, bool colored) {
    BatchPools p;
    p.path_pool = std::max<uint64_t>(l.path_pool, (uint64_t)nb / 2 + 128ull * g.paths + 1024);
    p.path_text = std::max<uint64_t>(l.path_text, (uint64_t)nb * FIRST_PATH_TEXT + (1u << 16));
    p.row_text = std::max<uint64_t>(l.row_text, (uint64_t)FIRST_ROW_TEXT * nb + (1u << 16));
    p.sites = std::max<uint64_t>(l.sites, (uint64_t)FIRST_SITES * nb + 64);
    p.groups = std::max<uint64_t>(l.groups, (uint64_t)FIRST_GROUPS * nb + 64);
    p.ilen = std::max<uint64_t>(l.ilen, (uint64_t)FIRST_ILEN * nb + 64);
    p.walk = colored ? std::max<uint64_t>(l.walk, (uint64_t)nb * 2 + 256ull * g.paths + 1024) : 0;
    return p;
}
inline uint64_t row_text_need(uint64_t path_text_used, uint32_t n_branching, uint32_t nb) { return 3 * path_text_used + 128ull * n_branching + 160ull * nb; }

inline uint64_t reserve_job_index_bytes(uint32_t nb) { return (uint64_t)nb / 4 * 4 + 4096; }
inline uint64_t reserve_site_values(uint32_t nb, const CallGrids &g) { return (uint64_t)nb / 4 + 1024ull * g.sites + 1024; }

}
```

Measured before the change: 242.1 million.

## Split alignment into strict and branching chains with separate counters and queues

Splits the call-alignment pipeline into two chains, strict and branching, each with its own counters, queue region and stack scratch slice, so the branching path/stack/sites work can run on the side stream while strict SNP/pair/stack tiers run on the main stream. The side-by-side mode is gated behind PF_ALIGN_CHAINS, and it defaults to off. When off, the branching work stays on the main stream, but it still uses separate counters and the new ordering. A PF_FIRST_POOLS_DIV knob can shrink the first-attempt pools. The change doubles the queue and stack scratch memory and adds extra host synchronisation points and retry bookkeeping.

```diff
diff --git a/ploidyfrost_amd/csrc/pf_call.hip b/ploidyfrost_amd/csrc/pf_call.hip
--- a/ploidyfrost_amd/csrc/pf_call.hip
+++ b/ploidyfrost_amd/csrc/pf_call.hip
@@ -390,14 +390,14 @@
 
 int ensure_batch_buffers(pf_ctx *ctx, const char *who, CallState::AlignWork &W, CallState::AlignOut &O, uint32_t nb) {
     const size_t list = (size_t)nb * 4;
-    return need(ctx, who, {{&W.counters, sizeof(CallCounters)}, {&W.btask, (size_t)nb * sizeof(pf_bubble_task)}, {&W.queues, (size_t)NQ * list},
+    return need(ctx, who, {{&W.counters, CALL_CHAINS * sizeof(CallCounters)}, {&W.btask, (size_t)nb * sizeof(pf_bubble_task)}, {&W.queues, chain_queue_entries(nb, NQ) * 4},
                            {&W.blist, list}, {&W.slist, list}, {&W.plist, list}, {&W.plist2, list}, {&W.klist, list}, {&W.klist_b, list}, {&W.has, list},
                            {&O.res, (size_t)nb * sizeof(pf_bubble_result)}, {&O.sv_off, (size_t)nb * 8}, {&O.vc, list}});
 }
 
 int ensure_wave_scratch(pf_ctx *ctx, const char *who, CallState::AlignWork &W, const CallGrids &g, uint32_t depth, bool stack_tier, bool pair_tier) {
     PF_TRY(need(ctx, who, {{&W.paths_scr, paths_per_wave(depth) * g.paths}}));
-    if (stack_tier) PF_TRY(need(ctx, who, {{&W.stack_scr, stack_scratch_bytes() * g.stack}}));
+    if (stack_tier) PF_TRY(need(ctx, who, {{&W.stack_scr, stack_scratch_total(stack_scratch_bytes(), g)}}));
     if (pair_tier) PF_TRY(need(ctx, who, {{&W.pair_scr, PairGeom<PAIR_MAX>::scratch_bytes * g.pair}}));
     return PF_OK;
 }
@@ -469,21 +469,29 @@
     const bool stack_tier = stack_scores(match, mismatch, gap);
     const int stack_ok = stack_tier ? std::max(1, std::min(3, env_int("PF_STACK_LEVEL", 1))) : 0;
     const int paths_force_scratch = env_int("PF_PATHS_SCRATCH", 0) ? 1 : 0;
+    const bool two_chains = env_int("PF_ALIGN_CHAINS", 0) != 0;
+    const uint32_t first_pools_div = (uint32_t)std::max(1, env_int("PF_FIRST_POOLS_DIV", 1));
     const CallGrids grids = call_grids(ctx->n_cu);
     const uint32_t depth;
-    hipStream_t st = nullptr;
-    CallCounters *d_cnt = nullptr;
+    hipStream_t st = nullptr, pst = nullptr, bst = nullptr;
+    CallCounters *d_cnt = nullptr, *d_cnt_b = nullptr;
     BatchRef batch = {};
     GraphSeq graph = {};
-    CallLists lists = {};
+    CallLists lists = {}, lists_b = {};
     RowPools pools;
     BatchPools cap = {};
+    PrepArgs pa = {};
     PathArgs ph = {};
     PairArgs pr = {};
     int attempt = 0;
-    CallCounters hc = {};
+    CallCounters hc = {}, hb = {};
     unsigned long long heads[4] = {0, 0, 0, 0};
     uint64_t n_jobs = 0;
+    int bubble_runs = 0;
+    bool sites_issued = false;
+    uint32_t sites_ks = 0;
+    uint64_t sites_sv_cap = 0;
+    int sites_sv_attempt = 0, sites_ks_attempt = 0;
     uint32_t n_called = 0;
     size_t tl_at = (size_t)-1;
 
@@ -501,10 +509,16 @@
         PF_TRY(ensure_wave_scratch(ctx, who, W, grids, depth, stack_tier, pair_tier));
         if (W.mlist_cap < MANY_LIST_MIN) W.mlist_cap = MANY_LIST_MIN;
         PF_TRY(need(ctx, who, {{&W.mlist, (size_t)W.mlist_cap * 4}}));
-        d_cnt = W.counters.as<CallCounters>();
+        pst = W.side_stream;
+        bst = two_chains ? pst : st;
+        d_cnt = W.counters.as<CallCounters>() + CHAIN_STRICT;
+        d_cnt_b = W.counters.as<CallCounters>() + CHAIN_BRANCHING;
         batch = BatchRef{S->ctask.as<CallTask>(), S->kept.as<uint32_t>(), t0, nb};
         graph = GraphSeq{ctx->d_seq, ctx->d_off, ctx->d_len};
         lists = CallLists{W.queues.as<uint32_t>(), W.blist.as<uint32_t>(), W.slist.as<uint32_t>(), W.plist.as<uint32_t>(), W.plist2.as<uint32_t>(), W.klist.as<uint32_t>(), W.klist_b.as<uint32_t>(), nb};
+        lists.queues += chain_queue_first(CHAIN_STRICT, nb, NQ);
+        lists_b = lists;
+        lists_b.queues = W.queues.as<uint32_t>() + chain_queue_first(CHAIN_BRANCHING, nb, NQ);
         trace.stage("lists and scratch");
         return PF_OK;
     }
@@ -514,37 +528,69 @@
         l.path_pool = S->path_pool; l.path_text = S->text_pool; l.row_text = S->otext_cap; l.sites = S->osites_cap; l.groups = S->ogroups_cap; l.ilen = S->oilen_cap;
         l.walk = W.walk_cap;
         cap = batch_pools(nb, grids, l, S->n_colors != 0);
+        if (first_pools_div > 1 && attempt == 0) cap.row_text = shrunk_pool(cap.row_text, first_pools_div, 64);
+        if (first_pools_div > 1 && attempt == 1) {
+            cap.sites = shrunk_pool(cap.sites, first_pools_div, 64); cap.groups = shrunk_pool(cap.groups, first_pools_div, 64);
+            cap.ilen = shrunk_pool(cap.ilen, first_pools_div, 64);
+        }
         PF_TRY(ensure_pools(ctx, who, W, O, nb, cap));
         unsigned long long *d_heads = bubble_pool_heads(ctx, lane);
         if (!d_heads) return PF_ERR_HIP;
         pools = RowPools{O.res.as<pf_bubble_result>(), O.otext.as<char>(), cap.row_text, O.osites.as<pf_bubble_site>(), cap.sites, O.ogroups.as<uint8_t>(), cap.groups,
                          O.oilen.as<uint32_t>(), cap.ilen, d_heads};
-        PF_HIP(hipMemsetAsync(d_cnt, 0, sizeof(CallCounters), st));
+        PF_HIP(hipMemsetAsync(W.counters.p, 0, CALL_CHAINS * sizeof(CallCounters), st));
         PF_HIP(hipMemsetAsync(d_heads, 0, 32, st));
-        return PF_OK;
-    }
-
-    int launch_tiers() {
-        PrepArgs pa;
+        sites_issued = false;
+        bubble_runs = 0;
+        n_jobs = 0;
+        return PF_OK;
+    }
+
+    int launch_prep() {
+        pa = PrepArgs{};
         pa.batch = batch; pa.len = graph.len; pa.btask = W.btask.as<pf_bubble_task>(); pa.bpath = W.bpath.as<pf_bubble_path>(); pa.res = pools.res;
         pa.lists = lists; pa.snp_ok = snp_ok ? 1 : 0; pa.pair_ok = pair_tier ? 1 : 0; pa.stack_ok = stack_ok; pa.cnt = d_cnt;
         tbegin(PF_K_CALL_PREP, st);
         k_call_prep<<<(nb + 255) / 256, 256, 0, st>>>(pa);
         tend(st);
-        hipStream_t pst = W.side_stream;
         PF_HIP(hipEventRecord(W.ev_prep, st));
         PF_HIP(hipStreamWaitEvent(pst, W.ev_prep, 0));
+        PF_HIP(hipMemcpyAsync(&d_cnt_b->n_branching, &d_cnt->n_branching, 4, hipMemcpyDeviceToDevice, pst));
+        return PF_OK;
+    }
+
+    int launch_paths() {
         ph = PathArgs{};
         ph.batch = batch; ph.blist = lists.blist; ph.succ = ctx->d_succ; ph.graph = graph; ph.k = ctx->k; ph.depth_cap = depth;
         ph.scratch = W.paths_scr.as<uint8_t>(); ph.scratch_per_wave = paths_per_wave(depth); ph.force_scratch = paths_force_scratch;
-        ph.max_paths = MAX_PATHS; ph.n_list = &d_cnt->n_branching; ph.mlist = W.mlist.as<uint32_t>(); ph.mlist_cap = W.mlist_cap;
+        ph.max_paths = MAX_PATHS; ph.n_list = &d_cnt_b->n_branching; ph.mlist = W.mlist.as<uint32_t>(); ph.mlist_cap = W.mlist_cap;
         ph.walk_pool = S->n_colors ? W.walk_pool.as<uint32_t>() : nullptr; ph.walk_off = W.walk_off.as<uint64_t>(); ph.walk_cap = cap.walk;
         ph.btask = pa.btask; ph.bpath = pa.bpath; ph.path_cap = cap.path_pool; ph.text = W.ptext.as<char>(); ph.text_cap = cap.path_text;
-        ph.queues = lists.queues; ph.klist = lists.klist_b; ph.stack_ok = stack_ok; ph.cnt = d_cnt;
+        ph.queues = lists_b.queues; ph.klist = lists.klist_b; ph.stack_ok = stack_ok; ph.cnt = d_cnt_b;
         tbegin(PF_K_CALL_PATHS, pst);
         k_call_paths<false><<<grids.paths, 64, 0, pst>>>(ph);
         tend(pst);
         PF_HIP(hipEventRecord(W.ev_paths, pst));
+        return PF_OK;
+    }
+
+    int launch_stack(int chain, hipStream_t s) {
+        if (!stack_tier) return PF_OK;
+        const bool branching = chain == CHAIN_BRANCHING;
+        StackArgs sk;
+        sk.list = branching ? lists.klist_b : lists.klist; sk.n_list = branching ? &d_cnt_b->n_stack_b : &d_cnt->n_stack;
+        sk.scratch = W.stack_scr.as<uint8_t>() + stack_scratch_first(chain, stack_scratch_bytes(), grids);
+        sk.pair_ok = branching ? 0 : pa.pair_ok;
+        sk.btask = pa.btask; sk.bpath = pa.bpath; sk.ptext = W.ptext.as<char>(); sk.graph = graph;
+        sk.M = (int)match; sk.D = (int)mismatch; sk.G = (int)gap;
+        sk.out = pools; sk.lists = branching ? lists_b : lists; sk.cnt = branching ? d_cnt_b : d_cnt;
+        tbegin(PF_K_CALL_STACK, s);
+        k_call_stack<<<grids.stack, 64, 0, s>>>(sk);
+        tend(s);
+        return PF_OK;
+    }
+
+    int launch_strict_tiers() {
         if (snp_ok) {
             SnpArgs sn;
             sn.batch = batch; sn.slist = lists.slist; sn.graph = graph; sn.out = pools; sn.lists = lists; sn.pair_ok = pa.pair_ok; sn.stack_ok = stack_ok; sn.cnt = d_cnt;
@@ -552,16 +598,7 @@
             k_call_snp<<<(nb + 255) / 256, 256, 0, st>>>(sn);
             tend(st);
         }
-        StackArgs sk;
-        if (stack_tier) {
-            sk.list = lists.klist; sk.n_list = &d_cnt->n_stack; sk.scratch = W.stack_scr.as<uint8_t>(); sk.pair_ok = pa.pair_ok;
-            sk.btask = pa.btask; sk.bpath = pa.bpath; sk.ptext = W.ptext.as<char>(); sk.graph = graph;
-            sk.M = (int)match; sk.D = (int)mismatch; sk.G = (int)gap;
-            sk.out = pools; sk.lists = lists; sk.cnt = d_cnt;
-            tbegin(PF_K_CALL_STACK, st);
-            k_call_stack<<<grids.stack, 64, 0, st>>>(sk);
-            tend(st);
-        }
+        PF_TRY(launch_stack(CHAIN_STRICT, st));
         if (pair_tier) {
             pr = PairArgs{};
             pr.batch = batch; pr.graph = graph; pr.M = match; pr.D = mismatch; pr.G = gap; pr.Mi = (int)match; pr.Di = (int)mismatch; pr.Gi = (int)gap;
@@ -577,21 +614,25 @@
             if (pair_stats) PF_TRY(print_pair_stats(ctx, prof));
             pr.prof = nullptr;
         }
-        PF_HIP(hipStreamWaitEvent(st, W.ev_paths, 0));
-        if (stack_tier) {
-            sk.list = lists.klist_b; sk.n_list = &d_cnt->n_stack_b; sk.pair_ok = 0;
-            tbegin(PF_K_CALL_STACK, st);
-            k_call_stack<<<grids.stack, 64, 0, st>>>(sk);
-            tend(st);
-        }
-        return PF_OK;
-    }
-
-    int read_counters() {
+        return PF_OK;
+    }
+
+    int read_strict() {
         PF_HIP(hipGetLastError());
         PF_HIP(hipMemcpyAsync(&hc, d_cnt, sizeof(hc), hipMemcpyDeviceToHost, st));
         PF_HIP(hipStreamSynchronize(st));
         return PF_OK;
+    }
+    int read_branching() {
+        PF_HIP(hipGetLastError());
+        PF_HIP(hipMemcpyAsync(&hb, d_cnt_b, sizeof(hb), hipMemcpyDeviceToHost, bst));
+        PF_HIP(hipStreamSynchronize(bst));
+        return PF_OK;
+    }
+    void drain() {
+        if (st) (void)hipStreamSynchronize(st);
+        if (pst) (void)hipStreamSynchronize(pst);
+        (void)hipGetLastError();
     }
 
     int launch_pair_tier2() {
@@ -610,58 +651,64 @@
             else k_call_pair<PAIR_MAX2, false><<<g2, 64, 0, st>>>(p2);
             tend(st);
         }
-        return read_counters();
+        return read_strict();
+    }
+
+    int finish_strict_tiers() {
+        PF_TRY(read_strict());
+        trace.stage(two_chains ? "strict: K-SNP .. K-PAIR done" : "K-PREP .. K-STACK done");
+        return launch_pair_tier2();
     }
 
     void note_units() const {
         ctx_units(ctx, PF_K_CALL_PREP, nb);
         if (snp_ok) ctx_units(ctx, PF_K_CALL_SNP, hc.n_snp);
         if (pair_tier) ctx_units(ctx, PF_K_CALL_PAIR, hc.n_pair + hc.n_pair2);
-        if (stack_tier) ctx_units(ctx, PF_K_CALL_STACK, hc.n_stack + hc.n_stack_b);
-        ctx_units(ctx, PF_K_CALL_PATHS, hc.n_branching);
-        if (trace.on) fprintf(stderr, "[pf_call_align] bubbles of more than 255 walks: %u, err %u\n", hc.n_many, hc.err);
+        if (stack_tier) ctx_units(ctx, PF_K_CALL_STACK, hc.n_stack + hb.n_stack_b);
+        ctx_units(ctx, PF_K_CALL_PATHS, hb.n_branching);
+        if (trace.on) fprintf(stderr, "[pf_call_align] bubbles of more than 255 walks: %u, err %u\n", hb.n_many, hb.err | hc.err);
     }
 
     int launch_paths_big(bool *retry) {
-        if (!hc.n_many || (hc.err & ERR_WALK)) return PF_OK;
-        if (hc.n_many > W.mlist_cap) {
-            W.mlist_cap = grown_many(hc.n_many);
+        if (!hb.n_many || (hb.err & ERR_WALK)) return PF_OK;
+        if (hb.n_many > W.mlist_cap) {
+            W.mlist_cap = grown_many(hb.n_many);
             *retry = true;
             return need(ctx, who, {{&W.mlist, (size_t)W.mlist_cap * 4}});
         }
-        const int big_grid = paths_big_grid(hc.n_many);
+        const int big_grid = paths_big_grid(hb.n_many);
         const uint64_t big_per_wave = paths_big_per_wave(depth, PATHS_BIG);
         PF_TRY(need(ctx, who, {{&W.paths_big_scr, big_per_wave * big_grid}}));
         PathArgs pb = ph;
-        pb.blist = W.mlist.as<uint32_t>(); pb.n_list = &d_cnt->n_many; pb.max_paths = PATHS_BIG; pb.mlist = nullptr; pb.mlist_cap = 0;
+        pb.blist = W.mlist.as<uint32_t>(); pb.n_list = &d_cnt_b->n_many; pb.max_paths = PATHS_BIG; pb.mlist = nullptr; pb.mlist_cap = 0;
         pb.scratch = W.paths_big_scr.as<uint8_t>(); pb.scratch_per_wave = big_per_wave;
-        tbegin(PF_K_CALL_PATHS, st);
-        k_call_paths<true><<<big_grid, 64, 0, st>>>(pb);
-        tend(st);
-        return read_counters();
+        tbegin(PF_K_CALL_PATHS, bst);
+        k_call_paths<true><<<big_grid, 64, 0, bst>>>(pb);
+        tend(bst);
+        return read_branching();
     }
 
     int accept_walks(bool *retry) {
-        if (hc.err & ERR_WALK) {
+        if (hb.err & ERR_WALK) {
             char where[96];
-            snprintf(where, sizeof where, " (superbubble from unitig %u%c to unitig %u%c)", (hc.err_entrance >> 1) + 1, (hc.err_entrance & 1) ? '-' : '+',
-                     (hc.err_exit >> 1) + 1, (hc.err_exit & 1) ? '-' : '+');
-            pf::CtxErr{ctx} = std::string(hc.err & ERR_MANY_PATHS ? "pf_call_run: a bubble has more than 65535 paths" : "pf_call_run: a bubble is deeper than the complex size allows") + where;
+            snprintf(where, sizeof where, " (superbubble from unitig %u%c to unitig %u%c)", (hb.err_entrance >> 1) + 1, (hb.err_entrance & 1) ? '-' : '+',
+                     (hb.err_exit >> 1) + 1, (hb.err_exit & 1) ? '-' : '+');
+            pf::CtxErr{ctx} = std::string(hb.err & ERR_MANY_PATHS ? "pf_call_run: a bubble has more than 65535 paths" : "pf_call_run: a bubble is deeper than the complex size allows") + where;
             return PF_ERR_ARG;
         }
         amax(S->otext_cap, cap.row_text); amax(S->osites_cap, cap.sites);
         amax(S->ogroups_cap, cap.groups); amax(S->oilen_cap, cap.ilen);
         amax(S->path_pool, cap.path_pool);
         amax(S->text_pool, cap.path_text);
-        const uint64_t rows_need = row_text_need(hc.text_head, hc.n_branching, nb);
+        const uint64_t rows_need = row_text_need(hb.text_head, hb.n_branching, nb);
         if (trace.on)
             fprintf(stderr, "[pf_call_align] attempt %d: %u bubbles, path pool %llu of %llu, path text %llu of %llu, rows text cap %llu (needs %llu)\n", attempt, nb,
-                    (unsigned long long)hc.path_head, (unsigned long long)cap.path_pool, (unsigned long long)hc.text_head, (unsigned long long)cap.path_text,
+                    (unsigned long long)hb.path_head, (unsigned long long)cap.path_pool, (unsigned long long)hb.text_head, (unsigned long long)cap.path_text,
                     (unsigned long long)cap.row_text, (unsigned long long)rows_need);
-        if (hc.path_head > cap.path_pool || hc.text_head > cap.path_text || hc.walk_head > cap.walk) {
-            amax(S->path_pool, grown(hc.path_head, 1024));
-            amax(S->text_pool, grown(hc.text_head, 4096));
-            if (S->n_colors) W.walk_cap = std::max<uint64_t>(W.walk_cap, grown(hc.walk_head, 1024));
+        if (hb.path_head > cap.path_pool || hb.text_head > cap.path_text || hb.walk_head > cap.walk) {
+            amax(S->path_pool, grown(hb.path_head, 1024));
+            amax(S->text_pool, grown(hb.text_head, 4096));
+            if (S->n_colors) W.walk_cap = std::max<uint64_t>(W.walk_cap, grown(hb.walk_head, 1024));
             *retry = true;
             return PF_OK;
         }
@@ -673,33 +720,44 @@
         return PF_OK;
     }
 
-    int run_bubble(bool *retry) {
-        n_jobs = 0;
-        for (int x = 0; x < NQ; ++x) n_jobs += hc.q_n[x];
-        PF_TRY(need(ctx, who, {{&W.scan_tmp2, std::max<size_t>((size_t)n_jobs, 1) * 4}}));
+    struct QueueSet { const CallCounters *h; const uint32_t *queues; };
+    static uint64_t jobs_of(const CallCounters &c) { uint64_t n = 0; for (int x = 0; x < NQ; ++x) n += c.q_n[x]; return n; }
+    int run_bubble(std::initializer_list<QueueSet> sets, hipStream_t s, const char *side) {
+        uint64_t jobs = 0;
+        for (const QueueSet &q : sets) jobs += jobs_of(*q.h);
+        PF_TRY(need(ctx, who, {{&W.scan_tmp2, std::max<size_t>((size_t)jobs, 1) * 4}}));
         uint32_t *d_idx = W.scan_tmp2.as<uint32_t>();
         size_t at = 0;
-        for (int x = 0; x < NQ; ++x) {
-            if (!hc.q_n[x]) continue;
-            PF_HIP(hipMemcpyAsync(d_idx + at, W.queues.as<uint32_t>() + (size_t)x * nb, (size_t)hc.q_n[x] * 4, hipMemcpyDeviceToDevice, st));
-            at += hc.q_n[x];
-        }
         BubbleLaunch BL;
+        for (int x = 0; x < NQ; ++x)
+            for (const QueueSet &q : sets) {
+                if (!q.h->q_n[x]) continue;
+                PF_HIP(hipMemcpyAsync(d_idx + at, q.queues + (size_t)x * nb, (size_t)q.h->q_n[x] * 4, hipMemcpyDeviceToDevice, s));
+                at += q.h->q_n[x];
+                BL.n_cls[x / 2] += q.h->q_n[x];
+            }
+        for (const QueueSet &q : sets) { BL.max_need = std::max<uint64_t>(BL.max_need, q.h->max_need); BL.retry_need = std::max<uint64_t>(BL.retry_need, q.h->retry_need); }
         BL.text = W.ptext.as<char>(); BL.paths = W.bpath.as<pf_bubble_path>(); BL.tasks = W.btask.as<pf_bubble_task>();
         BL.n_tasks = nb; BL.idx = d_idx;
-        for (int c = 0; c <= kBubLdsClasses; ++c) BL.n_cls[c] = hc.q_n[2 * c] + hc.q_n[2 * c + 1];
-        BL.max_need = hc.max_need; BL.retry_need = hc.retry_need;
         BL.match = match; BL.mismatch = mismatch; BL.gap = gap;
         BL.out = pools;
         BL.keep_heads = true;
-        BL.lane = lane; BL.stream = st;
-        trace.stage("K-BUBBLE launching");
-        const int bst = bubble_launch(ctx, BL, heads);
-        trace.stage("K-BUBBLE done");
+        BL.lane = lane; BL.stream = s;
+        trace.stage(two_chains ? (s == st ? "strict: K-BUBBLE launching" : "branching: K-BUBBLE launching") : "K-BUBBLE launching");
+        const int status = bubble_launch(ctx, BL, heads);
+        trace.stage(two_chains ? (s == st ? "strict: K-BUBBLE done" : "branching: K-BUBBLE done") : "K-BUBBLE done");
+        n_jobs += jobs;
+        ++bubble_runs;
         if (trace.on)
-            fprintf(stderr, "[pf_call_align] attempt %d: K-BUBBLE status %d, pools text %llu of %llu, sites %llu of %llu, groups %llu of %llu, indel lengths %llu of %llu\n", attempt, bst,
-                    heads[0], (unsigned long long)cap.row_text, heads[1], (unsigned long long)cap.sites, heads[2], (unsigned long long)cap.groups, heads[3], (unsigned long long)cap.ilen);
-        if (bst == PF_ERR_OVERFLOW && (heads[0] > cap.row_text || heads[1] > cap.sites || heads[2] > cap.groups || heads[3] > cap.ilen)) {
+            fprintf(stderr, "[pf_call_align] attempt %d: K-BUBBLE over %s: %llu jobs, status %d, pools text %llu of %llu, sites %llu of %llu, groups %llu of %llu, indel lengths %llu of %llu\n",
+                    attempt, side, (unsigned long long)jobs, status, heads[0], (unsigned long long)cap.row_text, heads[1], (unsigned long long)cap.sites, heads[2],
+                    (unsigned long long)cap.groups, heads[3], (unsigned long long)cap.ilen);
+        return status;
+    }
+
+    int settle_pools(int status, bool *retry) {
+        if (status != PF_OK && status != PF_ERR_OVERFLOW) return status;
+        if (heads[0] > cap.row_text || heads[1] > cap.sites || heads[2] > cap.groups || heads[3] > cap.ilen) {
             amax(S->otext_cap, heads[0] + heads[0] / 8);
             amax(S->osites_cap, heads[1] + heads[1] / 8);
             amax(S->ogroups_cap, heads[2] + heads[2] / 8);
@@ -707,7 +765,51 @@
             *retry = true;
             return PF_OK;
         }
-        return bst;
+        return status;
+    }
+
+    int attempt_serial(bool *retry) {
+        PF_TRY(launch_prep());
+        PF_TRY(launch_paths());
+        PF_TRY(launch_strict_tiers());
+        PF_HIP(hipStreamWaitEvent(st, W.ev_paths, 0));
+        PF_TRY(launch_stack(CHAIN_BRANCHING, st));
+        PF_TRY(read_branching());
+        PF_TRY(finish_strict_tiers());
+        note_units();
+        PF_TRY(launch_paths_big(retry));
+        if (!*retry) PF_TRY(accept_walks(retry));
+        if (*retry) return PF_OK;
+        const int status = run_bubble({{&hc, lists.queues}, {&hb, lists_b.queues}}, st, "both chains' queues");
+        return settle_pools(status, retry);
+    }
+
+    int attempt_chains(bool *retry) {
+        PF_TRY(launch_prep());
+        PF_TRY(launch_paths());
+        PF_TRY(launch_stack(CHAIN_BRANCHING, pst));
+        PF_TRY(launch_strict_tiers());
+        PF_TRY(read_branching());
+        trace.stage("branching: K-PATHS, K-STACK done");
+        PF_TRY(launch_paths_big(retry));
+        if (!*retry) PF_TRY(accept_walks(retry));
+        if (*retry) return PF_OK;
+        int status = PF_OK;
+        if (jobs_of(hb)) status = run_bubble({{&hb, lists_b.queues}}, bst, "the branching chain's queues");
+        if (status != PF_OK && status != PF_ERR_OVERFLOW) return status;
+        if (status == PF_OK && hb.n_branching) PF_TRY(sites_begin());
+        PF_TRY(finish_strict_tiers());
+        note_units();
+        if (status == PF_OK && jobs_of(hc)) {
+            status = run_bubble({{&hc, lists.queues}}, st, "the strict chain's queues");
+        } else {
+            unsigned long long *d_heads = bubble_pool_heads(ctx, lane);
+            if (!d_heads) return PF_ERR_HIP;
+            PF_HIP(hipMemcpyAsync(heads, d_heads, 32, hipMemcpyDeviceToHost, st));
+            PF_HIP(hipStreamSynchronize(st));
+        }
+        trace.stage("strict chain done");
+        return settle_pools(status, retry);
     }
 
     int number_called() {
@@ -724,7 +826,7 @@
         sa.k = ctx->k; sa.tab = ctx->d_tab; sa.mask = ctx->tab_cap - 1; sa.one_strand = ctx->tab_one_strand; sa.tab_exact = ctx->tab_exact;
         sa.low = S->low; sa.up = S->up; sa.ks = ks; sa.rows_cap = (uint32_t)rows_cap;
         sa.scratch = W.sites_scr.as<uint8_t>(); sa.scratch_per_wave = per_wave; sa.sv_off = O.sv_off.as<uint64_t>();
-        sa.sv = O.sv.as<double>(); sa.sv_cap = sv_cap; sa.cnt = d_cnt; sa.prof = nullptr;
+        sa.sv = O.sv.as<double>(); sa.sv_cap = sv_cap; sa.cnt = d_cnt_b; sa.prof = nullptr;
         sa.n_colors = S->n_colors;
         sa.ctab = CTab{ctx->d_ctab, ctx->ctab_cap - 1, ctx->ctab_line_bytes}; sa.c_one_strand = ctx->ctab_one_strand; sa.unread = ctx->d_unread;
         sa.clow = S->col_low.as<uint32_t>(); sa.cup = S->col_up.as<uint32_t>(); sa.full = S->col_full.as<uint64_t>(); sa.cwords = S->col_words;
@@ -734,53 +836,93 @@
         return sa;
     }
 
-    int launch_sites(SiteArgs &sa, int grid) {
+    int launch_sites() {
+        const uint32_t C = S->n_colors;
+        const uint64_t rows_cap = sites_rows_cap(hb.max_rows);
+        const uint64_t per_wave = sites_per_wave(rows_cap, sites_ks, C, S->col_words);
+        const int grid = call_sites_grid(hb.n_branching, grids, per_wave);
+        sites_sv_cap = site_values_cap(C, hb.n_branching, grid, S->sv_pool);
+        PF_TRY(need(ctx, who, {{&W.sites_scr, per_wave * grid}, {&O.sv, sites_sv_cap * 8}}));
+        SiteArgs sa = site_args(sites_ks, rows_cap, per_wave, sites_sv_cap);
         static const bool sites_stats = getenv("PF_SITES_STATS") != nullptr;
         DevTmp<unsigned long long> prof;
-        if (sites_stats) PF_TRY(stats_begin(ctx, prof, (size_t)grid * 6, st, &sa.prof));
-        PF_HIP(hipMemsetAsync(&d_cnt->sites_next, 0, 4, st));
-        PF_HIP(hipMemsetAsync(&d_cnt->sv_head, 0, 8, st));
-        PF_HIP(hipMemsetAsync(&d_cnt->site_strings, 0, 8, st));
-        tbegin(PF_K_CALL_SITES, st);
-        if (sa.n_colors) k_call_sites<true><<<grid, 64, 0, st>>>(sa);
-        else k_call_sites<false><<<grid, 64, 0, st>>>(sa);
-        tend(st);
-        ctx_units(ctx, PF_K_CALL_SITES, hc.n_branching);
-        if (sites_stats) { PF_HIP(hipGetLastError()); PF_TRY(print_sites_stats(ctx, prof, grid, st)); }
-        return read_counters();
-    }
-
-    int run_sites() {
-        uint32_t KS = std::max<uint32_t>(first_site_string(ctx->k), S->sites_ks.load());
-        const uint32_t C = S->n_colors;
-        const uint64_t rows_cap = sites_rows_cap(hc.max_rows);
-        for (int sv_attempt = 0, ks_attempt = 0;;) {
-            const uint64_t per_wave = sites_per_wave(rows_cap, KS, C, S->col_words);
-            const int grid = call_sites_grid(hc.n_branching, grids, per_wave);
-            const uint64_t sv_cap = site_values_cap(C, hc.n_branching, grid, S->sv_pool);
-            PF_TRY(need(ctx, who, {{&W.sites_scr, per_wave * grid}, {&O.sv, sv_cap * 8}}));
-            SiteArgs sa = site_args(KS, rows_cap, per_wave, sv_cap);
-            PF_TRY(launch_sites(sa, grid));
-            if (hc.err & ERR_SITE_LONG) {
-                if (++ks_attempt > 3 || hc.ks_need <= KS) { pf::CtxErr{ctx} = "pf_call_run: the room for a site string does not converge"; return PF_ERR_OVERFLOW; }
-                KS = grown_site_string(hc.ks_need);
-                amax(S->sites_ks, KS);
-                hc.err = 0; hc.ks_need = 0;
-                PF_HIP(hipMemsetAsync(&d_cnt->err, 0, 4, st));
-                PF_HIP(hipMemsetAsync(&d_cnt->ks_need, 0, 4, st));
+        if (sites_stats) PF_TRY(stats_begin(ctx, prof, (size_t)grid * 6, bst, &sa.prof));
+        PF_HIP(hipMemsetAsync(&d_cnt_b->sites_next, 0, 4, bst));
+        PF_HIP(hipMemsetAsync(&d_cnt_b->sv_head, 0, 8, bst));
+        PF_HIP(hipMemsetAsync(&d_cnt_b->site_strings, 0, 8, bst));
+        tbegin(PF_K_CALL_SITES, bst);
+        if (sa.n_colors) k_call_sites<true><<<grid, 64, 0, bst>>>(sa);
+        else k_call_sites<false><<<grid, 64, 0, bst>>>(sa);
+        tend(bst);
+        ctx_units(ctx, PF_K_CALL_SITES, hb.n_branching);
+        if (sites_stats) { PF_HIP(hipGetLastError()); PF_TRY(print_sites_stats(ctx, prof, grid, bst)); }
+        return PF_OK;
+    }
+
+    int sites_begin() {
+        sites_ks = std::max<uint32_t>(first_site_string(ctx->k), S->sites_ks.load());
+        sites_sv_attempt = sites_ks_attempt = 0;
+        PF_TRY(launch_sites());
+        sites_issued = true;
+        return PF_OK;
+    }
+    int sites_end() {
+        for (;;) {
+            PF_TRY(read_branching());
+            if (hb.err & ERR_SITE_LONG) {
+                if (++sites_ks_attempt > 3 || hb.ks_need <= sites_ks) { pf::CtxErr{ctx} = "pf_call_run: the room for a site string does not converge"; return PF_ERR_OVERFLOW; }
+                sites_ks = grown_site_string(hb.ks_need);
+                amax(S->sites_ks, sites_ks);
+                hb.err = 0; hb.ks_need = 0;
+                PF_HIP(hipMemsetAsync(&d_cnt_b->err, 0, 4, bst));
+                PF_HIP(hipMemsetAsync(&d_cnt_b->ks_need, 0, 4, bst));
+                PF_TRY(launch_sites());
                 continue;
             }
-            if (hc.err & ERR_MISSING_KMER) { pf::CtxErr{ctx} = "CDBG::readCov(): a kmer of a site string can not found ."; return PF_ERR_MISSING_KMER; }
-            if (hc.err & ERR_SITE_ROW) { pf::CtxErr{ctx} = "CDBG::PloidyEstimation(): a site string runs past the end of an aligned row (the reference terminates here: std::out_of_range from substr, src/CDBG.cpp:1478-1590)"; return PF_ERR_ARG; }
-            if (hc.err & ERR_SITE_UNITIG) { pf::CtxErr{ctx} = "CCDBG::PloidyEstimation(): a site string does not start on a unitig of its bubble"; return PF_ERR_ARG; }
-            if (hc.sv_head > sv_cap) {
-                if (sv_attempt++ >= 2) { pf::CtxErr{ctx} = "pf_call_run: site value pool does not converge"; return PF_ERR_OVERFLOW; }
-                amax(S->sv_pool, grown(hc.sv_head, 1024));
+            if (hb.err & ERR_MISSING_KMER) { pf::CtxErr{ctx} = "CDBG::readCov(): a kmer of a site string can not found ."; return PF_ERR_MISSING_KMER; }
+            if (hb.err & ERR_SITE_ROW) { pf::CtxErr{ctx} = "CDBG::PloidyEstimation(): a site string runs past the end of an aligned row (the reference terminates here: std::out_of_range from substr, src/CDBG.cpp:1478-1590)"; return PF_ERR_ARG; }
+            if (hb.err & ERR_SITE_UNITIG) { pf::CtxErr{ctx} = "CCDBG::PloidyEstimation(): a site string does not start on a unitig of its bubble"; return PF_ERR_ARG; }
+            if (hb.sv_head > sites_sv_cap) {
+                if (sites_sv_attempt++ >= 2) { pf::CtxErr{ctx} = "pf_call_run: site value pool does not converge"; return PF_ERR_OVERFLOW; }
+                amax(S->sv_pool, grown(hb.sv_head, 1024));
+                PF_TRY(launch_sites());
                 continue;
             }
-            amax(S->sv_pool, sv_cap);
+            amax(S->sv_pool, sites_sv_cap);
             return PF_OK;
         }
+    }
+
+    int run(pf_call_result *out) {
+        PF_TRY(prepare());
+        for (attempt = 0;; ++attempt) {
+            if (attempt > 5) { pf::CtxErr{ctx} = "pf_call_align: pools do not converge"; return PF_ERR_OVERFLOW; }
+            bool retry = false;
+            PF_TRY(size_pools());
+            PF_TRY(two_chains ? attempt_chains(&retry) : attempt_serial(&retry));
+            if (!retry) break;
+            drain();
+        }
+        out->n_branching = hb.n_branching;
+        const unsigned int stack_done = hc.n_stack_done + hb.n_stack_done;
+        out->align_jobs = n_jobs + hc.n_snp_done + hc.n_pair_done + hc.n_pair2_done + stack_done;
+        out->snp_jobs = hc.n_snp_done; out->pair_jobs = hc.n_pair_done + hc.n_pair2_done; out->wave_jobs = n_jobs; out->stack_jobs = stack_done;
+        if (trace.on)
+            fprintf(stderr, "[pf_call_align] chains %s: %u branching bubbles, K-BUBBLE jobs %llu (branching chain) + %llu (strict chain) in %d runs\n",
+                    two_chains ? "side by side" : "one behind the other", hb.n_branching, (unsigned long long)jobs_of(hb), (unsigned long long)jobs_of(hc), bubble_runs);
+        PF_TRY(number_called());
+        if (hb.n_branching) {
+            if (!sites_issued) PF_TRY(sites_begin());
+            PF_TRY(sites_end());
+        } else {
+            PF_TRY(need(ctx, who, {{&O.sv, 16}}));
+        }
+        if (two_chains) trace.stage("branching chain done");
+        trace.stage("K-SITES done");
+        PF_HIP(hipStreamSynchronize(st));
+        out->site_strings = hb.site_strings;
+        out->n_called = n_called;
+        return PF_OK;
     }
 };
 
@@ -802,39 +944,13 @@
     if (t1 - t0 > (1u << 24)) { pf::CtxErr{ctx} = "pf_call_align: at most 2^24 bubbles per batch"; return PF_ERR_ARG; }
     PF_HIP(hipSetDevice(ctx->device));
     AlignCall A(ctx, lane, t0, (uint32_t)(t1 - t0), complex_size, match, mismatch, gap);
-    PF_TRY(A.prepare());
-    for (A.attempt = 0;; ++A.attempt) {
-        if (A.attempt > 5) { pf::CtxErr{ctx} = "pf_call_align: pools do not converge"; return PF_ERR_OVERFLOW; }
-        bool retry = false;
-        PF_TRY(A.size_pools());
-        PF_TRY(A.launch_tiers());
-        PF_TRY(A.read_counters());
-        A.trace.stage("K-PREP .. K-STACK done");
-        PF_TRY(A.launch_pair_tier2());
-        A.note_units();
-        PF_TRY(A.launch_paths_big(&retry));
-        if (!retry) PF_TRY(A.accept_walks(&retry));
-        if (!retry) PF_TRY(A.run_bubble(&retry));
-        if (!retry) break;
-    }
-    const CallCounters &hc = A.hc;
-    out->n_branching = hc.n_branching;
-    out->align_jobs = A.n_jobs + hc.n_snp_done + hc.n_pair_done + hc.n_pair2_done + hc.n_stack_done;
-    out->snp_jobs = hc.n_snp_done; out->pair_jobs = hc.n_pair_done + hc.n_pair2_done; out->wave_jobs = A.n_jobs; out->stack_jobs = hc.n_stack_done;
-    PF_TRY(A.number_called());
-    if (hc.n_branching) {
-        PF_TRY(A.run_sites());
-    } else {
-        PF_TRY(need(ctx, A.who, {{&O.sv, 16}}));
-        PF_HIP(hipStreamSynchronize(A.st));
-    }
-    out->site_strings = hc.site_strings;
-    A.trace.stage("K-SITES done");
-    out->n_called = A.n_called;
+    const int status = A.run(out);
+    if (status != PF_OK) { A.drain(); return status; }
+    const CallCounters &hb = A.hb;
     O.nb = A.nb;
     O.cur = *out;
     for (int x = 0; x < 4; ++x) O.used[x] = A.heads[x];
-    O.used[4] = hc.n_branching ? hc.sv_head : 0;
+    O.used[4] = hb.n_branching ? hb.sv_head : 0;
     return PF_OK;
 }
 
diff --git a/ploidyfrost_amd/csrc/pf_call_plan.hpp b/ploidyfrost_amd/csrc/pf_call_plan.hpp
--- a/ploidyfrost_amd/csrc/pf_call_plan.hpp
+++ b/ploidyfrost_amd/csrc/pf_call_plan.hpp
@@ -24,6 +24,14 @@
 inline int paths_big_grid(uint32_t n_many) { return (int)std::min<uint32_t>(n_many, 32); }
 constexpr uint32_t MANY_LIST_MIN = 4096;
 inline uint32_t grown_many(uint32_t n_many) { return n_many + n_many / 8 + 64; }
+
+constexpr int CALL_CHAINS = 2;
+enum Chain : int { CHAIN_STRICT = 0, CHAIN_BRANCHING = 1 };
+inline uint64_t chain_queue_entries(uint32_t nb, int n_queues) { return (uint64_t)CALL_CHAINS * n_queues * nb; }
+inline uint64_t chain_queue_first(int chain, uint32_t nb, int n_queues) { return (uint64_t)chain * n_queues * nb; }
+inline uint64_t stack_scratch_total(uint64_t per_wave, const CallGrids &g) { return (uint64_t)CALL_CHAINS * per_wave * g.stack; }
+inline uint64_t stack_scratch_first(int chain, uint64_t per_wave, const CallGrids &g) { return (uint64_t)chain * per_wave * g.stack; }
+inline uint64_t shrunk_pool(uint64_t cap, uint32_t div, uint64_t least) { return div > 1 ? std::max<uint64_t>(cap / div, least) : cap; }
 
 inline int call_pair2_grid(uint32_t n_pair2, const CallGrids &g) { return (int)std::min<uint32_t>((n_pair2 + 63) / 64, (uint32_t)g.pair2); }
 inline uint32_t pair2_min(int n_cu) { return (uint32_t)n_cu * 32u; }
```

After: 237.7 million. 1.8% lower.
